# nikhilTkur/Multigrid_Nikhil_C-

Measured on AMD Instinct MI355X. Metric: fine_grid_stencil_updates_per_sec, higher is better.
Workload: dtype f64

## Files before the change

multigrid_nikhil_c-_amd/csrc/mgx.hip:

```cpp

#include "../../include/mgx.h"
#include "mgx_bottom.hpp"
#include "mgx_kernels.hpp"
#include "mgx_launch.hpp"
#include "mgx_var.hpp"
#include "mgx_galerkin.hpp"
#include "mgx_opdep.hpp"
#include "mgx_cheby.hpp"
#include "mgx_line.hpp"
#include "mgx_colour.hpp"
#include "mgx_small.hpp"
#include "mgx_krylov.hpp"
#include "mgx_refine.hpp"
#include "mgx_refine_gcr.hpp"
#include "mgx_multi.hpp"
#include "mgx_eig.hpp"
#include "mgx_eig_many.hpp"
#include "mgx_dist_plan.hpp"

#include <chrono>
#include <unistd.h>
#include <cmath>
#include <cstdio>
#include <cstdlib>
#include <cstring>
#include <string>
#include <vector>

namespace {

using namespace mgx;

thread_local std::string g_create_error;

void log_runtime_libs(const char* where)
{
    if (env_int("MGX_LOG_RUNTIME_LIBS", 0) == 0) return;
    char buf[8192];
    if (mgx_runtime_libs(buf, sizeof buf) >= 0)
        std::fprintf(stderr, "[mgx] runtime libraries mapped at %s (pid %d):\n%s", where, (int)getpid(), buf);
}

struct Level {
    int L = 0, N = 0, rows = 0;
    long pitch = 0;
    size_t bytes = 0;
    bool f64 = true;
    void *u = nullptr, *b = nullptr, *tmp = nullptr, *r = nullptr;
    void* A[9] = {};
    void* J[9] = {};
    void* wt[8] = {nullptr, nullptr, nullptr, nullptr, nullptr, nullptr, nullptr, nullptr};
    bool nine = false;
    bool stencil_set = false;
    void* cheb = nullptr;
    double lambda_g = 0.0;
    void *line_m[2] = {nullptr, nullptr}, *line_g[2] = {nullptr, nullptr}, *line_hf = nullptr, *line_hb = nullptr;
    int line_R = 0;
    size_t esize() const { return f64 ? 8 : 4; }
};

struct EventPair { hipEvent_t a, b; int cls; long long launches; long long sweeps; hipEvent_t a_use; };

}

struct mgx_solver {
    mgx_config cfg{};
    hipStream_t stream = nullptr;
    std::vector<Level> lv;
    Level fine64;
    bool mixed = false;
    bool work_f64 = true;
    BottomDST bottom;
    double* partial = nullptr;
    long partial_cap = 0;
    double* sum_dev = nullptr;
    double* sum_host = nullptr;
    std::string err;
    int rows_per_chunk = 0;
    FuseCfg fuse{10, 0, 256, 10, 10, 1024, 10, 10};
    std::vector<EventPair> ev_used, ev_free;
    double prof_ms[MGX_PROF_COUNT] = {0};
    long long prof_launches[MGX_PROF_COUNT] = {0};
    long long prof_sweeps[MGX_PROF_COUNT] = {0};
    int last_smooth_launches = 0;
    int fold = 1;
    int use_zero_in = 1;
    int norm_blocks_ready = 0;
    double fine_updates = 0.0;
    struct CycleGraph {
        std::vector<void*> before, after;
        hipGraphExec_t exec = nullptr;
        double fine_updates = 0.0;
    };
    std::vector<CycleGraph> graphs;
    int use_graph = 1;
    bool prof_mute = false;
    bool prof_chain = false;
    hipEvent_t chain_ev = nullptr;
    int mixed_fuse = 1;
    double *var_M = nullptr, *var_inv = nullptr, *var_pm = nullptr, *var_pi = nullptr;
    bool var = false;
    bool galerkin = false;
    bool gal_built = false;
    int cycle = MGX_CYCLE_V;
    int small_visit = 1;
    int small_max_n = kSmallMaxN;
    int line_dirs = 0;
    int colour = 0;
    int gs_fused = 1;
    int* line_flag = nullptr;
    int transfer = MGX_TRANSFER_BILINEAR;
    struct KrylovWs {
        void *x = nullptr, *b = nullptr;
        void *p[2] = {nullptr, nullptr}, *q = nullptr;
        void *Z[kGcrMaxRestart] = {}, *Q[kGcrMaxRestart] = {};
        double* part = nullptr;
        long part_cap = 0;
        double *sc = nullptr, *sc_host = nullptr;
        int vecs(mgx_solver* s, std::initializer_list<void**> vs, size_t bytes);
        int shared(mgx_solver* s, size_t bytes, int blocks);
        void free();
    } kry;
    struct mgx_dist* dist = nullptr;
    mgx_solver* shadow = nullptr;
    long long op_gen = 0, shadow_gen = -1;
    bool own_stream = true;
    struct MultiWs {
        struct Grids { void *u[MGX_MAX_RHS] = {}, *tmp[MGX_MAX_RHS] = {}, *b[MGX_MAX_RHS] = {}, *r[MGX_MAX_RHS] = {}; };
        std::vector<Grids> lv;
        double* part[MGX_MAX_RHS] = {};
        double *sums = nullptr, *sums_host = nullptr;
        int cols = 0;
        void* x[MGX_MAX_RHS] = {};
        void *Z[MGX_MAX_RHS][kGcrMaxRestart] = {}, *Q[MGX_MAX_RHS][kGcrMaxRestart] = {};
        double* gpart[MGX_MAX_RHS] = {};
        double *gsc = nullptr, *gsc_host = nullptr;
    } multi;
    struct EigWs {
        void *X[MGX_MAX_RHS] = {}, *AX[MGX_MAX_RHS] = {}, *AW[MGX_MAX_RHS] = {}, *P[MGX_MAX_RHS] = {}, *AP[MGX_MAX_RHS] = {};
        double *gpart = nullptr, *gsum = nullptr, *gsum_host = nullptr;
        int cols = 0;
    } eig;
    struct EigManyWs {
        void* Y[MGX_EIGS_MAX] = {};
        void** ytab = nullptr;
        double *coef = nullptr, *part = nullptr;
        int slots = 0;
    } eigm;

    int fail(int code, const std::string& m) { err = m; return code; }
};

namespace {

#define HIPCHK(h, expr)                                                                  \
    do {                                                                                 \
        hipError_t e__ = (expr);                                                         \
        if (e__ != hipSuccess)                                                           \
            return (h)->fail(MGX_ERR_HIP, std::string(#expr) + ": " + hipGetErrorString(e__)); \
    } while (0)

struct Prof {
    mgx_solver* s; int idx = -1;
    Prof(mgx_solver* s_, int cls, long long launches, bool on = true) : s(s_)
    {
        static const bool mute_all = env_int("MGX_PROF_MUTE", 0) != 0;
        if (!on || !s->cfg.profile || s->prof_mute || mute_all) return;
        EventPair p;
        if (!s->ev_free.empty()) { p = s->ev_free.back(); s->ev_free.pop_back(); }
        else {
            static const unsigned flags = env_int("MGX_PROF_EVENT_FLAGS", 1) ? hipEventDisableSystemFence : hipEventDefault;
            if (hipEventCreateWithFlags(&p.a, flags) != hipSuccess || hipEventCreateWithFlags(&p.b, flags) != hipSuccess) return;
        }
        p.cls = cls; p.launches = launches; p.sweeps = 0;
        p.a_use = p.a;
        if (s->prof_chain && s->chain_ev) p.a_use = s->chain_ev;
        else (void)hipEventRecord(p.a, s->stream);
        s->ev_used.push_back(p);
        idx = (int)s->ev_used.size() - 1;
    }
    void set(long long launches, long long sweeps)
    {
        if (idx >= 0) { s->ev_used[idx].launches = launches; s->ev_used[idx].sweeps = sweeps; }
    }
    ~Prof()
    {
        if (idx < 0) return;
        (void)hipEventRecord(s->ev_used[idx].b, s->stream);
        if (s->prof_chain) s->chain_ev = s->ev_used[idx].b;
    }
};

int prof_collect(mgx_solver* s)
{
    if (s->ev_used.empty()) return MGX_OK;
    HIPCHK(s, hipStreamSynchronize(s->stream));
    for (auto& p : s->ev_used) {
        float ms = 0.f;
        if (hipEventElapsedTime(&ms, p.a_use, p.b) == hipSuccess) {
            s->prof_ms[p.cls] += ms;
            s->prof_launches[p.cls] += p.launches;
            s->prof_sweeps[p.cls] += p.sweeps;
        }
        s->ev_free.push_back(p);
    }
    s->ev_used.clear();
    s->chain_ev = nullptr;
    return MGX_OK;
}

template <typename T>
__global__ void k_fill_rhs(T* b, int N, long pitch, int kind, double f)
{
    const int c = blockIdx.x * blockDim.x + threadIdx.x;
    const int r = blockIdx.y;
    if (c > N || r > N) return;
    const double h = 1.0 / (double)N;
    double v = 0.0;
    if (r >= 1 && r < N && c >= 1 && c < N) {
        if (kind == 0) v = f * h * h;
        else v = h * h * 8.0 * 9.869604401089358 * sinpi(2.0 * c * h) * sinpi(2.0 * r * h);
    }
    b[(long)r * pitch + c] = (T)v;
}

__device__ inline uint64_t splitmix64(uint64_t x)
{
    x += 0x9E3779B97F4A7C15ULL;
    x = (x ^ (x >> 30)) * 0xBF58476D1CE4E5B9ULL;
    x = (x ^ (x >> 27)) * 0x94D049BB133111EBULL;
    return x ^ (x >> 31);
}

template <typename T>
__global__ void k_fill_random(T* u, int N, long pitch, uint64_t seed)
{
    const int c = blockIdx.x * blockDim.x + threadIdx.x;
    const int r = blockIdx.y;
    if (c > N || r > N) return;
    double v = 0.0;
    if (r >= 1 && r < N && c >= 1 && c < N) {
        const uint64_t idx = (uint64_t)(r - 1) * (uint64_t)(N - 1) + (uint64_t)(c - 1);
        const uint64_t x = splitmix64(seed ^ splitmix64(idx));
        v = (double)(x >> 11) * (1.0 / 4503599627370496.0) - 1.0;
    }
// ... 503 lines not shown
    return fold_eligible(s, s->lv[level], s->cfg.mu1, false, 1, true);
}

bool smooth_folded(mgx_solver* s, int level, int mu, bool pre, int post, bool zero_in = false, bool coarse_zero_in = false)
{
    Level& l = s->lv[level];
    if (!fold_eligible(s, l, mu, pre, post)) return false;
    const bool fine = (level == s->cfg.finest_level);
    const bool rbgs = (s->cfg.smoother == MGX_SMOOTHER_RBGS);
    if (!l.f64 && !rbgs && mu == 10 && l.N > s->fuse.tile_max_n && post == 2 && pre &&
        cycle_k_supported(mu, false, false, 0, pre, s->fuse.arith) && !cycle_k_supported(mu, false, false, post, pre, s->fuse.arith))
        post = 0;
    {
        Prof p(s, fine ? MGX_PROF_SMOOTH_FINE : MGX_PROF_COARSE, mu);
        const Level& c = s->lv[level - 1];
        const int dt = l.f64 ? MGX_DTYPE_F64 : MGX_DTYPE_F32;
        const mgx_slab cs{level - 1, dt, c.rows, 0, s->cfg.arith};
        void* czero = (post == 1 && coarse_zero_in) ? nullptr : c.u;
        const BlockReq q = level_req(s, l, mu, pre, post, zero_in, env_int("MGX_ROWS", 0));
        int launches = 0;
        const int nb = with_kernel_set(l.f64, s->cfg.smoother, s->fuse.arith, [&](auto k) {
            using K = decltype(k);
            using T = typename K::T;
            return fold_block<T, K::SM, K::AR>(s->fuse, q, (T*)l.u, (const T*)l.b, (T*)l.tmp, l.pitch, s->cfg.omega, &cs,
                                               pre ? (const T*)c.u : nullptr, post == 1 ? (T*)c.b : nullptr, (T*)czero, 1, c.N,
                                               s->cfg.restrict_mode, s->partial, s->stream, &launches);
        });
        if (nb < 0) return false;
        if (launches & 1) std::swap(l.u, l.tmp);
        p.set(launches, mu);
        if (post == 2) s->norm_blocks_ready = nb;
    }
    if (fine) s->fine_updates += (double)mu * (double)(l.N - 1) * (double)(l.N - 1);
    return true;
}

void smooth_t(mgx_solver* s, Level& l, int mu)
{
    int launches = 0;
    with_kernel_set(l.f64, s->cfg.smoother, s->fuse.arith, [&](auto k) {
        using K = decltype(k);
        using T = typename K::T;
        (void)fold_block<T, K::SM, K::AR>(s->fuse, level_req(s, l, mu, false, 0, false, s->rows_per_chunk), (T*)l.u, (const T*)l.b,
                                          (T*)l.tmp, l.pitch, s->cfg.omega, nullptr, nullptr, nullptr, nullptr, 0, 0, 0, nullptr,
                                          s->stream, &launches);
    });
    s->last_smooth_launches = launches;
    if (launches & 1) std::swap(l.u, l.tmp);
}

void smooth(mgx_solver* s, int level, int mu, bool post = false, const MultiSet& a = kOwnSet, double* fu = nullptr)
{
    if (mu <= 0) return;
    Level& l = s->lv[level];
    const bool fine = (level == s->cfg.finest_level);
    Prof p(s, fine ? MGX_PROF_SMOOTH_FINE : MGX_PROF_COARSE, mu, own(a));
    if (s->var) smooth_var(s, level, a, mu, post);
    else smooth_t(s, l, mu);
    p.set(s->last_smooth_launches, mu);
    if (!fine) return;
    const double updates = (double)(s->line_dirs == 3 ? 2 * mu : mu) * (double)(l.N - 1) * (double)(l.N - 1);
    if (own(a)) s->fine_updates += updates;
    else if (fu) for (int j = 0; j < a.m; ++j) fu[a.act[j]] += updates;
}

void restrict_level(mgx_solver* s, int level, bool fused, bool zero_guess, const MultiSet& a = kOwnSet)
{
    Level& f = s->lv[level];
    Level& c = s->lv[level - 1];
    const bool fine = (level == s->cfg.finest_level);
    Prof p(s, fine ? MGX_PROF_RESTRICT_FINE : MGX_PROF_COARSE, 1, own(a));
    const int rpc = s->rows_per_chunk;
    const int mode = s->cfg.restrict_mode;
    with_float_type(f.f64, [&](auto tag) {
        using T = decltype(tag);
        const SetPtrs<const T> uf = set_ptrs<const T>(s, level, a, kU), bf = set_ptrs<const T>(s, level, a, kB);
        const SetPtrs<T> cb = set_ptrs<T>(s, level - 1, a, kB);
        const SetPtrs<T> cz = zero_guess ? set_ptrs<T>(s, level - 1, a, kU) : SetPtrs<T>{};
        if (opdep(s)) {
            const Launch g = make_launch(c.N, VecOf<T>::W, c.N - 1, 1);
            const T rscale = (mode == MGX_RESTRICT_FW16) ? (T)0.25 : (T)1;
            const dim3 grd(g.blocks), blk(kBlock);
            if (!fused) hipLaunchKernelGGL((k_restrict_opdep<T, 0>), grd, blk, 0, s->stream, uf.p[0], bf.p[0], op9_of<T>(f), wt8_of<T>(c), cb.p[0],
                                           cz.p[0], c.N, f.pitch, c.pitch, g.strips, rscale);
            else with_point_count(f.nine, [&](auto nq) {
                constexpr int MODE = decltype(nq)::value == 9 ? 2 : 1;
                if (a.m == 1) hipLaunchKernelGGL((k_restrict_opdep<T, MODE>), grd, blk, 0, s->stream, uf.p[0], bf.p[0], op9_of<T>(f), wt8_of<T>(c),
                                                 cb.p[0], cz.p[0], c.N, f.pitch, c.pitch, g.strips, rscale);
                else with_count<kMultiMax, 2>(a.m, [&](auto kc) {
                    constexpr int K = decltype(kc)::value;
                    hipLaunchKernelGGL((k_restrict_opdep_multi<T, MODE, K>), grd, blk, 0, s->stream, columns_in<K>(uf.p), columns_in<K>(bf.p),
                                       op9_of<T>(f), wt8_of<T>(c), columns_out<K>(cb.p), columns_out<K>(cz.p), c.N, f.pitch, c.pitch, g.strips, rscale);
                });
            });
            return;
        }
        const bool grid_residual = fused && (s->var || mode >= MGX_RESTRICT_INJECT);
        if (grid_residual) {
            if (s->var) residual_set<T, 0>(s, level, a);
            else residual_level<0>(s, f, f.u, f.b, f.r);
        }
        const SetPtrs<const T> src = grid_residual ? set_ptrs<const T>(s, level, a, kR) : bf;
        for (int j = 0; j < a.m; ++j) {
            if (mode >= MGX_RESTRICT_INJECT) {
                const double w = (mode == MGX_RESTRICT_INJECT4) ? 4.0 : 1.0;
                const dim3 blk(256), grd((c.N + 255) / 256, c.N - 1);
                hipLaunchKernelGGL((k_restrict_inject<T>), grd, blk, 0, s->stream, src.p[j], cb.p[j], cz.p[j], c.N, f.pitch, c.pitch, (T)w);
            } else {
                launch_restrict<T>(uf.p[j], src.p[j], cb.p[j], cz.p[j], f.N, f.pitch, c.pitch, 1, c.N, 0, mode, fused && !grid_residual, rpc, s->stream);
            }
        }
    });
}

void prolong_level(mgx_solver* s, int level, bool add, const MultiSet& a = kOwnSet)
{
    Level& f = s->lv[level];
    Level& c = s->lv[level - 1];
    const bool fine = (level == s->cfg.finest_level);
    Prof p(s, fine ? MGX_PROF_PROLONG_FINE : MGX_PROF_COARSE, 1, own(a));
    with_float_type(f.f64, [&](auto tag) {
        using T = decltype(tag);
        const SetPtrs<T> v = set_ptrs<T>(s, level, a, kU);
        const SetPtrs<const T> e = set_ptrs<const T>(s, level - 1, a, kU);
        if (opdep(s)) launch_prolong_opdep<T>(a.m, add, v.p, e.p, wt8_of<T>(c), c.N, f.pitch, c.pitch, s->stream);
        else for (int j = 0; j < a.m; ++j) launch_prolong<T>(v.p[j], e.p[j], f.N, f.pitch, c.pitch, 1, f.N, 0, add, s->rows_per_chunk, s->stream);
    });
}

void bottom_solve(mgx_solver* s, const MultiSet& a = kOwnSet)
{
    const int level = s->cfg.coarsest_level;
    Level& l = s->lv[level];
    Prof p(s, (l.L == s->cfg.finest_level) ? MGX_PROF_SMOOTH_FINE : MGX_PROF_COARSE, 4, own(a));
    const int n = l.N - 1;
    with_float_type(l.f64, [&](auto tag) {
        using T = decltype(tag);
        const SetPtrs<const T> b = set_ptrs<const T>(s, level, a, kB);
        const SetPtrs<T> u = set_ptrs<T>(s, level, a, kU);
        if (s->var) launch_var_dense_solve<T>(s->var_inv, a.m, b.p, u.p, n, l.pitch, s->stream);
        else s->bottom.solve<T>(b.p[0], u.p[0], l.pitch, s->stream);
    });
}

int zero_u(mgx_solver* s, int level, const MultiSet& a = kOwnSet)
{
    for (int j = 0; j < a.m; ++j) HIPCHK(s, hipMemsetAsync(slot(s, level, a.act[j], kU), 0, s->lv[level].bytes, s->stream));
    return MGX_OK;
}

bool descend(mgx_solver* s, int level, bool zero_in_here, const MultiSet& a = kOwnSet, double* fu = nullptr)
{
    const bool zin_next = own(a) && zero_in_ok(s, level - 1);
    if (!own(a) || !smooth_folded(s, level, s->cfg.mu1, false, 1, zero_in_here, zin_next)) {
        if (zero_in_here) (void)zero_u(s, level, a);
        smooth(s, level, s->cfg.mu1, false, a, fu);
        restrict_level(s, level, true, !zin_next, a);
    }
    return zin_next;
}

void ascend(mgx_solver* s, int level, int post, const MultiSet& a = kOwnSet, double* fu = nullptr)
{
    if (!own(a) || !smooth_folded(s, level, s->cfg.mu2, true, post)) {
        prolong_level(s, level, true, a);
        smooth(s, level, s->cfg.mu2, true, a, fu);
    }
}

void vcycle(mgx_solver* s, int level, bool zero_in_here = false, int post_top = 0, int kind = -1, const MultiSet& a = kOwnSet,
            double* fu = nullptr);

bool small_level(const mgx_solver* s, int level, const MultiSet& a)
{
    if (!own(a) || !s->small_visit || s->cycle == MGX_CYCLE_V || !s->galerkin || !s->gal_built) return false;
    if (s->cfg.smoother != MGX_SMOOTHER_JACOBI) return false;
    if (level <= s->cfg.coarsest_level || level >= s->cfg.finest_level) return false;
    const Level& l = s->lv[level];
    return l.nine && l.N <= s->small_max_n;
}

void small_visit(mgx_solver* s, int level, bool ascend, bool descend)
{
    Level& f = s->lv[level];
    Level& c = s->lv[level - 1];
    Prof p(s, MGX_PROF_COARSE, 1);
    with_float_type(f.f64, [&](auto tag) {
        using T = decltype(tag);
        SmallVisit<T> a;
        a.u = (T*)f.u; a.b = (const T*)f.b;
        a.a = op9_of<T>(f); a.r = jac9_of<T>(f); a.dinv = (const T*)f.J[0];
        a.cu = (T*)c.u; a.cb = (T*)c.b;
        a.w = wt8_of<T>(c);
        a.N = f.N; a.pitch = f.pitch; a.cpitch = c.pitch;
        a.ascend = ascend; a.descend = descend; a.mu1 = s->cfg.mu1; a.mu2 = s->cfg.mu2;
        a.opdep = opdep(s);
        a.omega = (T)s->cfg.omega;
        a.rc = (T)(1.0 - (double)a.omega);
        const bool fw16 = s->cfg.restrict_mode == MGX_RESTRICT_FW16;
        a.rscale = fw16 ? (T)0.25 : (T)1;
        a.wgt = fw16 ? (T)0.0625 : (T)0.25;
        launch_small_visit<T>(a, s->stream);
    });
    p.set(1, (ascend ? s->cfg.mu2 : 0) + (descend ? s->cfg.mu1 : 0));
}

void coarse_visits(mgx_solver* s, int level, bool zero_in_here, int kind, const MultiSet& a = kOwnSet, double* fu = nullptr)
{
    const bool twice = kind != MGX_CYCLE_V && level > s->cfg.coarsest_level;
    const int second = kind == MGX_CYCLE_F ? MGX_CYCLE_V : kind;
    if (twice && small_level(s, level, a)) {
        small_visit(s, level, false, true);
        coarse_visits(s, level - 1, false, kind);
        small_visit(s, level, true, true);
        coarse_visits(s, level - 1, false, second);
        small_visit(s, level, true, false);
        return;
    }
    vcycle(s, level, zero_in_here, 0, kind, a, fu);
    if (twice) vcycle(s, level, false, 0, second, a, fu);
}

void vcycle(mgx_solver* s, int level, bool zero_in_here, int post_top, int kind, const MultiSet& a, double* fu)
{
    if (kind < 0) kind = s->cycle;
    if (level == s->cfg.coarsest_level) {
        if (s->cfg.bottom == MGX_BOTTOM_EXACT) {
            bottom_solve(s, a);
        } else {
            smooth(s, level, s->cfg.mu1, false, a, fu);
            smooth(s, level, s->cfg.mu2, true, a, fu);
        }
        return;
    }
    if (small_level(s, level, a)) {
        small_visit(s, level, false, true);
        coarse_visits(s, level - 1, false, kind);
        small_visit(s, level, true, false);
        return;
    }
    const bool zin_next = descend(s, level, zero_in_here, a, fu);
    coarse_visits(s, level - 1, zin_next, kind, a, fu);
    ascend(s, level, post_top, a, fu);
}

int fmg(mgx_solver* s)
{
    const int lo = s->cfg.coarsest_level, hi = s->cfg.finest_level;
    for (int l = hi; l > lo; --l) restrict_level(s, l, false, false);
    if (s->cfg.bottom == MGX_BOTTOM_EXACT) {
        bottom_solve(s);
    } else {
        int rc = zero_u(s, lo);
        if (rc) return rc;
        for (int i = 0; i <= s->cfg.mu0; ++i) vcycle(s, lo);
    }
    for (int l = lo + 1; l <= hi; ++l) {
        prolong_level(s, l, false);
        for (int i = 0; i <= s->cfg.mu0; ++i) vcycle(s, l);
    }
    return MGX_OK;
}

int enqueue_norm(mgx_solver* s, const Level& l, const void* u, const void* b, int cls)
{
    if (s->norm_blocks_ready > 0 && u == s->lv[s->cfg.finest_level].u && !s->mixed) {
        Prof p(s, cls, 1);
        hipLaunchKernelGGL(k_reduce_partials, dim3(1), dim3(kReduceThreads), 0, s->stream, s->partial, s->norm_blocks_ready,
                           s->sum_dev);
    } else {
        Prof p(s, cls, 2);
        residual_level<1>(s, l, u, b, nullptr);
    }
    s->norm_blocks_ready = 0;
    HIPCHK(s, hipMemcpyAsync(s->sum_host, s->sum_dev, sizeof(double), hipMemcpyDeviceToHost, s->stream));
    return MGX_OK;
}

int residual_norm_grid(mgx_solver* s, const Level& l, const void* u, const void* b, double* out, int cls)
{
    int rc = enqueue_norm(s, l, u, b, cls);
    if (rc) return rc;
    HIPCHK(s, hipStreamSynchronize(s->stream));
    *out = std::sqrt(*s->sum_host);
    return MGX_OK;
}

constexpr size_t kMaxGraphs = 8;

std::vector<void*> buffer_state(const mgx_solver* s)
{
    std::vector<void*> v;
    for (int l = s->cfg.coarsest_level; l <= s->cfg.finest_level; ++l) { v.push_back(s->lv[l].u); v.push_back(s->lv[l].tmp); }
    return v;
}

void set_buffer_state(mgx_solver* s, const std::vector<void*>& v)
{
    size_t i = 0;
    for (int l = s->cfg.coarsest_level; l <= s->cfg.finest_level; ++l) { s->lv[l].u = v[i++]; s->lv[l].tmp = v[i++]; }
}

template <typename Body>
hipGraphExec_t cached_graph(mgx_solver* s, unsigned tag, Body&& enqueue)
{
    std::vector<void*> key = buffer_state(s);
    key.push_back(reinterpret_cast<void*>((uintptr_t)tag));
    for (auto& c : s->graphs)
        if (c.before == key) {
            set_buffer_state(s, c.after);
            s->fine_updates += c.fine_updates;
            return c.exec;
        }
    if (s->graphs.size() >= kMaxGraphs) return nullptr;
    const double fu0 = s->fine_updates;
    hipGraph_t graph = nullptr;
    hipGraphExec_t exec = nullptr;
    hipError_t e = hipStreamBeginCapture(s->stream, hipStreamCaptureModeThreadLocal);
    if (e == hipSuccess) {
        s->prof_mute = true;
        const int rc = enqueue();
        s->prof_mute = false;
        e = hipStreamEndCapture(s->stream, &graph);
        if (e == hipSuccess && rc != MGX_OK) e = hipErrorUnknown;
        if (e == hipSuccess) e = hipGraphInstantiate(&exec, graph, nullptr, nullptr, 0);
        if (graph) (void)hipGraphDestroy(graph);
    }
    if (e != hipSuccess) {
        (void)hipGetLastError();
        set_buffer_state(s, key);
        s->fine_updates = fu0;
        s->use_graph = 0;
        return nullptr;
    }
    s->graphs.push_back({key, buffer_state(s), exec, s->fine_updates - fu0});
    return exec;
}

int coarse_part_graph(mgx_solver* s, int level, bool zero_in_here)
{
    auto body = [&] { coarse_visits(s, level, zero_in_here, s->cycle); return MGX_OK; };
    const hipGraphExec_t exec = cached_graph(s, 4u | (zero_in_here ? 8u : 0u), body);
    if (!exec) return body();
    Prof p(s, MGX_PROF_COARSE, 1);
    HIPCHK(s, hipGraphLaunch(exec, s->stream));
    return MGX_OK;
}

int zero_start_u(mgx_solver* s, bool* implicit)
{
    const int L = s->cfg.finest_level;
    const bool one_level = L == s->cfg.coarsest_level;
    *implicit = zero_in_ok(s, L);
    if (*implicit) return MGX_OK;
    if (one_level && !s->mixed) return MGX_OK;
    return zero_u(s, L);
}

int enqueue_cycle(mgx_solver* s, bool want_norm, bool zero_start, bool split)
{
    struct Chain {
        mgx_solver* s;
        Chain(mgx_solver* s_, bool on) : s(s_) { s->prof_chain = on && env_int("MGX_PROF_CHAIN", 1) != 0; s->chain_ev = nullptr; }
        ~Chain() { s->prof_chain = false; s->chain_ev = nullptr; }
    } chain(s, split);
    const int L = s->cfg.finest_level;
    const int post = want_norm ? 2 : 0;
    s->norm_blocks_ready = 0;
    bool zin = false;
    if (zero_start)
        if (int rc = zero_start_u(s, &zin)) return rc;
    if (split) {
        const bool zin_next = descend(s, L, zin);
        if (int rc = coarse_part_graph(s, L - 1, zin_next)) return rc;
        ascend(s, L, post);
    } else {
        vcycle(s, L, zin, post);
    }
    return want_norm ? enqueue_norm(s, s->lv[L], s->lv[L].u, s->lv[L].b, MGX_PROF_NORM_FINE) : MGX_OK;
}

int cycle_body(mgx_solver* s, bool want_norm, bool zero_start, double* r)
{
    const bool split = s->cfg.profile == 2 && s->use_graph && !s->mixed && s->cfg.finest_level > s->cfg.coarsest_level;
    const bool whole = s->use_graph && !s->cfg.profile && !s->mixed;
    auto body = [&] { return enqueue_cycle(s, want_norm, zero_start, split); };
    const hipGraphExec_t exec = whole ? cached_graph(s, (want_norm ? 1u : 0u) | (zero_start ? 2u : 0u), body) : nullptr;
    if (exec) {
        s->norm_blocks_ready = 0;
        HIPCHK(s, hipGraphLaunch(exec, s->stream));
    } else if (int rc = body()) {
        return rc;
    }
    if (!want_norm) return MGX_OK;
    HIPCHK(s, hipStreamSynchronize(s->stream));
    *r = std::sqrt(*s->sum_host);
    return MGX_OK;
}

void finish_solve(mgx_stats* stats, double* history, int history_cap, const std::vector<double>& hist, int cycles, bool converged,
                  std::chrono::steady_clock::time_point t0, double fine_updates)
{
    if (stats) {
        stats->cycles = cycles;
        stats->initial_residual = hist.front();
        stats->final_residual = hist.back();
        stats->converged = converged ? 1 : 0;
        stats->seconds = std::chrono::duration<double>(std::chrono::steady_clock::now() - t0).count();
        stats->fine_updates = fine_updates;
        stats->history_len = (int)hist.size();
    }
    if (history)
        for (int i = 0; i < (int)hist.size() && i < history_cap; ++i) history[i] = hist[i];
}

double pow2_floor(double x)
{
    int e;
    (void)std::frexp(x, &e);
    return std::ldexp(1.0, e - 1);
}

Level* pick(mgx_solver* s, int level, int which, void** grid)
{
    Level* l = &s->lv[level];
    if (s->mixed && level == s->cfg.finest_level) l = &s->fine64;
    switch (which) {
        case MGX_VEC_U: *grid = l->u; break;
        case MGX_VEC_B: *grid = l->b; break;
        case MGX_VEC_R: *grid = l->r; break;
        default: *grid = nullptr;
    }
    return l;
}

template <typename T>
void fold_ring(std::vector<T>& b, const T* ring, size_t n)
{
    const size_t N = n + 1;
    const T* top = ring;
    const T* bot = ring + (N + 1);
    const T* lef = ring + 2 * (N + 1);
    const T* rig = lef + (N - 1);
    for (size_t j = 0; j < n; ++j) {
        b[j] += top[j + 1];
        b[(n - 1) * n + j] += bot[j + 1];
    }
    for (size_t i = 0; i < n; ++i) {
        b[i * n] += lef[i];
        b[i * n + (n - 1)] += rig[i];
    }
}

template <typename Enqueue>
int time_on_stream(mgx_solver* s, double* ms, Enqueue enqueue)
{
    hipEvent_t a = nullptr, b = nullptr;
    auto timed = [&]() -> int {
        HIPCHK(s, hipEventCreate(&a));
        HIPCHK(s, hipEventCreate(&b));
        HIPCHK(s, hipEventRecord(a, s->stream));
        enqueue();
        HIPCHK(s, hipEventRecord(b, s->stream));
        HIPCHK(s, hipEventSynchronize(b));
        HIPCHK(s, hipGetLastError());
        float f = 0.f;
        HIPCHK(s, hipEventElapsedTime(&f, a, b));
        *ms = f;
        return MGX_OK;
    };
    const int rc = timed();
    if (a) (void)hipEventDestroy(a);
    if (b) (void)hipEventDestroy(b);
    return rc;
}

}

#include "mgx_dist.hpp"

#define NO_DIST(s)                                                                        \
    if ((s)->dist) return (s)->fail(MGX_ERR_STATE, "not available on a multi-GPU handle (see mgx.h, Multi-GPU)");

#include "mgx_krylov_host.hpp"
#include "mgx_multi_host.hpp"

static int create_solver(const mgx_config* cfg, const mgx_solver* like, mgx_handle* out);

#include "mgx_refine_host.hpp"
#include "mgx_multi_refine_host.hpp"
#include "mgx_eig_host.hpp"
#include "mgx_eig_many_host.hpp"

extern "C" {

int mgx_config_default(mgx_config* c)
{
    if (!c) return MGX_ERR_INVALID;
    c->finest_level = 10;
    c->coarsest_level = 7;
    c->mu0 = 30;
    c->mu1 = 10;
    c->mu2 = 10;
    c->omega = 2.0 / 3.0;
    c->smoother = MGX_SMOOTHER_JACOBI;
    c->dtype = MGX_DTYPE_F64;
    c->schedule = MGX_SCHEDULE_FMG;
    c->restrict_mode = MGX_RESTRICT_CONSISTENT;
    c->bottom = MGX_BOTTOM_EXACT;
    c->device = 0;
    c->profile = 0;
    c->n_gpus = 0;
    c->cut_level = 0;
    for (int i = 0; i < MGX_MAX_GPUS; ++i) c->devices[i] = -1;
    c->arith = MGX_ARITH_SEPARATE;
    c->op = MGX_OPERATOR_POISSON;
    return MGX_OK;
}

const char* mgx_status_string(int st)
{
    switch (st) {
        case MGX_OK: return "ok";
        case MGX_ERR_INVALID: return "invalid argument";
        case MGX_ERR_NO_DEVICE: return "no usable HIP device";
        case MGX_ERR_HIP: return "HIP runtime error";
        case MGX_ERR_ALLOC: return "device allocation failed";
        case MGX_ERR_STATE: return "invalid state";
        default: return "unknown status";
    }
}

const char* mgx_last_error(mgx_handle h) { return h ? h->err.c_str() : g_create_error.c_str(); }

int mgx_level_n(int level) { return (level >= 1 && level < 31) ? (1 << level) - 1 : -1; }

long mgx_level_pitch(int level, int dtype)
{
    if (level < 1 || level > 20 || (dtype != MGX_DTYPE_F32 && dtype != MGX_DTYPE_F64)) return -1;
    return level_pitch(level, dtype);
}

static int create_solver(const mgx_config* cfg, const mgx_solver* like, mgx_handle* out)
{
    if (!cfg || !out) { g_create_error = "null argument"; return MGX_ERR_INVALID; }
    *out = nullptr;
    if (cfg->coarsest_level < 2 || cfg->finest_level < cfg->coarsest_level || cfg->finest_level > 15 ||
        cfg->mu0 < 0 || cfg->mu1 < 0 || cfg->mu2 < 0 || !(cfg->omega > 0.0 && cfg->omega < 2.0) ||
        cfg->smoother < 0 || cfg->smoother > MGX_SMOOTHER_COLOR_SGS || cfg->smoother == 3 || cfg->smoother == 7 || cfg->dtype < 0 || cfg->dtype > 2 ||
        cfg->schedule < 0 || cfg->schedule > 1 || cfg->restrict_mode < 0 || cfg->restrict_mode > MGX_RESTRICT_INJECT4 ||
        cfg->bottom < 0 || cfg->bottom > 1 || cfg->arith < 0 || cfg->arith > 1 || (cfg->op != MGX_OPERATOR_POISSON && cfg->op != MGX_OPERATOR_STENCIL5 && cfg->op != MGX_OPERATOR_GALERKIN)) {
        g_create_error = "invalid configuration";
        return MGX_ERR_INVALID;
    }
    const bool galerkin = (cfg->op == MGX_OPERATOR_GALERKIN);
    const bool var = (cfg->op == MGX_OPERATOR_STENCIL5) || galerkin;
    if (cfg->bottom == MGX_BOTTOM_EXACT && cfg->coarsest_level > (var ? 5 : 8)) {
        g_create_error = var ? "exact bottom solve of a general operator (dense inverse) supports coarsest_level <= 5"
                             : "exact bottom solve supports coarsest_level <= 8";
        return MGX_ERR_INVALID;
    }
    const bool cheby = (cfg->smoother == MGX_SMOOTHER_CHEBYSHEV);
    if (cheby && !var) {
        g_create_error = "MGX_SMOOTHER_CHEBYSHEV: op = MGX_OPERATOR_STENCIL5 or MGX_OPERATOR_GALERKIN only (the constant stencil has its fused and folded passes)";
        return MGX_ERR_INVALID;
    }
    const bool line = (cfg->smoother >= MGX_SMOOTHER_LINE_X && cfg->smoother <= MGX_SMOOTHER_LINE_ALT);
    const bool colour = (cfg->smoother == MGX_SMOOTHER_COLOR_GS || cfg->smoother == MGX_SMOOTHER_COLOR_SGS);
    if (colour && (!var || cfg->dtype == MGX_DTYPE_MIXED || cfg->arith != MGX_ARITH_SEPARATE || cfg->n_gpus > 1)) {
        g_create_error = "MGX_SMOOTHER_COLOR_GS / COLOR_SGS: op = MGX_OPERATOR_STENCIL5 or MGX_OPERATOR_GALERKIN, dtype F64 or F32, arith SEPARATE, one GPU";
        return MGX_ERR_INVALID;
    }
    if (line && (!var || cfg->dtype == MGX_DTYPE_MIXED || cfg->arith != MGX_ARITH_SEPARATE || cfg->n_gpus > 1)) {
        g_create_error = "MGX_SMOOTHER_LINE_X / LINE_Y / LINE_ALT: op = MGX_OPERATOR_STENCIL5 or MGX_OPERATOR_GALERKIN, dtype F64 or F32, arith SEPARATE, one GPU";
        return MGX_ERR_INVALID;
    }
    if (var && (cfg->dtype == MGX_DTYPE_MIXED || cfg->smoother == MGX_SMOOTHER_RBGS || cfg->arith != MGX_ARITH_SEPARATE || cfg->n_gpus > 1)) {
// ... 369 lines not shown

int mgx_set_coefficient(mgx_handle s, const double* a_nodes, size_t count)
{
    if (!s || !a_nodes) return MGX_ERR_INVALID;
    NO_DIST(s)
    if (!s->var) return s->fail(MGX_ERR_STATE, "handle was created with op = MGX_OPERATOR_POISSON");
    const int Lf = s->cfg.finest_level, Nf = 1 << Lf;
    if (count != (size_t)(Nf + 1) * (size_t)(Nf + 1)) return s->fail(MGX_ERR_INVALID, "coefficient must hold (N + 1)^2 nodal values, N = 2^finest_level");
    double* dev = nullptr;
    if (hipMalloc(&dev, count * sizeof(double)) != hipSuccess) return s->fail(MGX_ERR_ALLOC, "hipMalloc failed for the nodal coefficient");
    int rc = MGX_OK;
    if (hipMemcpyAsync(dev, a_nodes, count * sizeof(double), hipMemcpyHostToDevice, s->stream) != hipSuccess) rc = s->fail(MGX_ERR_HIP, "copy of the nodal coefficient failed");
    for (int lv = s->galerkin ? Lf : s->cfg.coarsest_level; lv <= Lf && rc == MGX_OK; ++lv) {
        Level& l = s->lv[lv];
        const dim3 blk(256), grd((l.N + 1 + 255) / 256, l.N + 1);
        const int q = 1 << (Lf - lv);
        with_float_type(l.f64, [&](auto tag) {
            using T = decltype(tag);
            hipLaunchKernelGGL((k_var_from_nodes<T>), grd, blk, 0, s->stream, dev, Nf, q, out9(op9_of<T>(l)), l.N, l.pitch);
        });
        if (!s->galerkin) rc = var_build(s, l);
    }
    if (hipStreamSynchronize(s->stream) != hipSuccess && rc == MGX_OK) rc = s->fail(MGX_ERR_HIP, "sampling the nodal coefficient failed");
    (void)hipFree(dev);
    if (s->galerkin && rc == MGX_OK) { s->lv[Lf].nine = false; galerkin_invalidate(s); }
    return rc;
}

int mgx_get_stencil(mgx_handle s, int level, int which, void* dst, size_t count)
{
    if (!s || !dst) return MGX_ERR_INVALID;
    NO_DIST(s)
    if (!s->var) return s->fail(MGX_ERR_STATE, "handle was created with op = MGX_OPERATOR_POISSON");
    if (!level_ok(s, level) || which < 0 || which > 9) return s->fail(MGX_ERR_INVALID, "level or array selector out of range");
    Level& l = s->lv[level];
    if (l.nine) return s->fail(MGX_ERR_STATE, "nine-point operator (a coarse level, or a nine-point finest level, of a GALERKIN handle): use mgx_get_stencil9");
    if (!l.stencil_set) return s->fail(MGX_ERR_STATE, "operator of this level not set");
    if (s->galerkin && which >= 5 && !s->gal_built) return s->fail(MGX_ERR_STATE, "Galerkin hierarchy not built (mgx_build_galerkin)");
    return copy_out(s, l, which < 5 ? l.A[which] : l.J[which - 5], dst, count);
}

int mgx_build_galerkin(mgx_handle s)
{
    if (!s) return MGX_ERR_INVALID;
    NO_DIST(s)
    if (!s->galerkin) return s->fail(MGX_ERR_STATE, "handle was not created with op = MGX_OPERATOR_GALERKIN");
    if (!s->lv[s->cfg.finest_level].stencil_set)
        return s->fail(MGX_ERR_STATE, "finest operator not set (mgx_set_stencil / mgx_set_coefficient / mgx_set_stencil9 / mgx_set_tensor)");
    return s->work_f64 ? galerkin_build_t<double>(s, MGX_TRANSFER_BILINEAR) : galerkin_build_t<float>(s, MGX_TRANSFER_BILINEAR);
}

int mgx_build_galerkin_transfer(mgx_handle s, int transfer)
{
    if (!s) return MGX_ERR_INVALID;
    NO_DIST(s)
    if (!s->galerkin) return s->fail(MGX_ERR_STATE, "handle was not created with op = MGX_OPERATOR_GALERKIN");
    if (transfer != MGX_TRANSFER_BILINEAR && transfer != MGX_TRANSFER_OPERATOR)
        return s->fail(MGX_ERR_INVALID, "transfer must be MGX_TRANSFER_BILINEAR or MGX_TRANSFER_OPERATOR");
    if (!s->lv[s->cfg.finest_level].stencil_set)
        return s->fail(MGX_ERR_STATE, "finest operator not set (mgx_set_stencil / mgx_set_coefficient / mgx_set_stencil9 / mgx_set_tensor)");
    return s->work_f64 ? galerkin_build_t<double>(s, transfer) : galerkin_build_t<float>(s, transfer);
}

int mgx_get_transfer(mgx_handle s, int* transfer)
{
    if (!s || !transfer) return MGX_ERR_INVALID;
    NO_DIST(s)
    if (!s->galerkin) return s->fail(MGX_ERR_STATE, "handle was not created with op = MGX_OPERATOR_GALERKIN");
    if (!s->gal_built) return s->fail(MGX_ERR_STATE, "Galerkin hierarchy not built (mgx_build_galerkin)");
    *transfer = s->transfer;
    return MGX_OK;
}

int mgx_get_lambda_max(mgx_handle s, int level, double* out)
{
    if (!s || !out) return MGX_ERR_INVALID;
    NO_DIST(s)
    if (!s->var) return s->fail(MGX_ERR_STATE, "handle was created with op = MGX_OPERATOR_POISSON (g = 2 for the constant stencil)");
    if (!level_ok(s, level)) return s->fail(MGX_ERR_INVALID, "level out of range");
    if (s->galerkin && !s->gal_built) return s->fail(MGX_ERR_STATE, "Galerkin hierarchy not built (mgx_build_galerkin)");
    if (!s->lv[level].stencil_set) return s->fail(MGX_ERR_STATE, "operator of this level not set");
    *out = s->lv[level].lambda_g;
    return MGX_OK;
}

int mgx_get_line_factor(mgx_handle s, int level, int dir, int which, void* dst, size_t count)
{
    if (!s || !dst) return MGX_ERR_INVALID;
    NO_DIST(s)
    if (!s->line_dirs) return s->fail(MGX_ERR_STATE, "handle was not created with a line smoother (MGX_SMOOTHER_LINE_X / LINE_Y / LINE_ALT)");
    if (!level_ok(s, level) || dir < 0 || dir > 1 || which < 0 || which > 1) return s->fail(MGX_ERR_INVALID, "level, direction or array selector out of range");
    if (!(s->line_dirs & (1 << dir))) return s->fail(MGX_ERR_STATE, dir == 0 ? "the handle's smoother has no x-lines (MGX_SMOOTHER_LINE_Y)" : "the handle's smoother has no y-lines (MGX_SMOOTHER_LINE_X)");
    if (s->galerkin && !s->gal_built) return s->fail(MGX_ERR_STATE, "Galerkin hierarchy not built (mgx_build_galerkin)");
    if (!s->lv[level].stencil_set) return s->fail(MGX_ERR_STATE, "operator of this level not set");
    Level& l = s->lv[level];
    return copy_out(s, l, which == 0 ? l.line_m[dir] : l.line_g[dir], dst, count);
}

int mgx_get_line_chunks(mgx_handle s, int level, int* rows, int* chunks)
{
    if (!s || !rows || !chunks) return MGX_ERR_INVALID;
    NO_DIST(s)
    if (!(s->line_dirs & 2)) return s->fail(MGX_ERR_STATE, "the handle's smoother has no y-lines (MGX_SMOOTHER_LINE_Y / LINE_ALT)");
    if (!level_ok(s, level)) return s->fail(MGX_ERR_INVALID, "level out of range");
    *rows = s->lv[level].line_R;
    *chunks = line_chunks(s->lv[level].N, s->lv[level].line_R);
    return MGX_OK;
}

int mgx_get_prolongation(mgx_handle s, int level, int which, void* dst, size_t count)
{
    if (!s || !dst) return MGX_ERR_INVALID;
    NO_DIST(s)
    if (!s->galerkin) return s->fail(MGX_ERR_STATE, "handle was not created with op = MGX_OPERATOR_GALERKIN");
    if (level <= s->cfg.coarsest_level || level > s->cfg.finest_level || which < 0 || which > 7)
        return s->fail(MGX_ERR_INVALID, "level or array selector out of range");
    if (!s->gal_built) return s->fail(MGX_ERR_STATE, "Galerkin hierarchy not built (mgx_build_galerkin)");
    if (s->transfer != MGX_TRANSFER_OPERATOR)
        return s->fail(MGX_ERR_STATE, "the hierarchy was built with MGX_TRANSFER_BILINEAR: its weights are 1/2 and 1/4 and are not stored");
    Level& c = s->lv[level - 1];
    return copy_out(s, c, c.wt[which], dst, count);
}

int mgx_get_stencil9(mgx_handle s, int level, int which, void* dst, size_t count)
{
    if (!s || !dst) return MGX_ERR_INVALID;
    NO_DIST(s)
    if (!s->galerkin) return s->fail(MGX_ERR_STATE, "handle was not created with op = MGX_OPERATOR_GALERKIN");
    if (!level_ok(s, level) || which < 0 || which > 17) return s->fail(MGX_ERR_INVALID, "level or array selector out of range");
    if (!s->gal_built) return s->fail(MGX_ERR_STATE, "Galerkin hierarchy not built (mgx_build_galerkin)");
    Level& l = s->lv[level];
    const void* src = which < 9 ? l.A[which] : l.J[which - 9];
    const int slot = which < 9 ? which : which - 9;
    if (!src || (!l.nine && slot >= 5)) {
        const size_t n = (size_t)l.N - 1;
        if (count != n * n) return s->fail(MGX_ERR_INVALID, "vector length must be n*n with n = 2^level - 1");
        std::memset(dst, 0, count * l.esize());
        return MGX_OK;
    }
    return copy_out(s, l, src, dst, count);
}

#define MIXED_GUARD(lvl)                                                                  \
    if (s->mixed && (lvl) == s->cfg.finest_level)                                         \
        return s->fail(MGX_ERR_STATE, "dtype MIXED: operators and schedules are not defined on the finest level " \
                                      "(double data, float inner cycle); use mgx_solve, or a F64 / F32 handle");

#define OP_PROLOGUE(lvl_min)                                                              \
    if (!s) return MGX_ERR_INVALID;                                                       \
    NO_DIST(s)                                                                            \
    if (level < (lvl_min) || level > s->cfg.finest_level)                                 \
        return s->fail(MGX_ERR_INVALID, "level out of range for this operator");          \
    MIXED_GUARD(level)                                                                    \
    if (int vr__ = var_ready(s, s->cfg.coarsest_level, level)) return vr__;

#define OP_EPILOGUE                                                                       \
    HIPCHK(s, hipGetLastError());                                                         \
    HIPCHK(s, hipStreamSynchronize(s->stream));                                           \
    return MGX_OK;

int mgx_smooth(mgx_handle s, int level, int mu)
{
    OP_PROLOGUE(s->cfg.coarsest_level)
    if (mu < 0) return s->fail(MGX_ERR_INVALID, "mu must be >= 0");
    smooth(s, level, mu);
    OP_EPILOGUE
}

int mgx_residual(mgx_handle s, int level)
{
    OP_PROLOGUE(s->cfg.coarsest_level)
    Level& l = s->lv[level];
    int rc = ensure_r(s, l);
    if (rc) return rc;
    residual_level<0>(s, l, l.u, l.b, l.r);
    OP_EPILOGUE
}

int mgx_restrict(mgx_handle s, int level)
{
    OP_PROLOGUE(s->cfg.coarsest_level + 1)
    restrict_level(s, level, true, true);
    OP_EPILOGUE
}

int mgx_restrict_rhs(mgx_handle s, int level)
{
    OP_PROLOGUE(s->cfg.coarsest_level + 1)
    restrict_level(s, level, false, false);
    OP_EPILOGUE
}

int mgx_prolong_add(mgx_handle s, int level)
{
    OP_PROLOGUE(s->cfg.coarsest_level + 1)
    prolong_level(s, level, true);
    OP_EPILOGUE
}

int mgx_prolong(mgx_handle s, int level)
{
    OP_PROLOGUE(s->cfg.coarsest_level + 1)
    prolong_level(s, level, false);
    OP_EPILOGUE
}

int mgx_bottom_solve(mgx_handle s)
{
    if (!s) return MGX_ERR_INVALID;
    NO_DIST(s)
    if (s->cfg.bottom != MGX_BOTTOM_EXACT) return s->fail(MGX_ERR_STATE, "handle was created with bottom = SMOOTH");
    MIXED_GUARD(s->cfg.coarsest_level)
    if (int vr = var_ready(s, s->cfg.coarsest_level, s->cfg.coarsest_level)) return vr;
    bottom_solve(s);
    OP_EPILOGUE
}

int mgx_residual_norm(mgx_handle s, int level, double* out)
{
    if (!s || !out) return MGX_ERR_INVALID;
    if (!level_ok(s, level)) return s->fail(MGX_ERR_INVALID, "level out of range");
    if (s->dist) {
        if (level != s->cfg.finest_level) return s->fail(MGX_ERR_STATE, "multi-GPU handles: residual norm of the finest level only");
        return dist_norm(s, s->dist, out);
    }
    if (int vr = var_ready(s, level, level)) return vr;
    void* gu = nullptr; void* gb = nullptr;
    Level* l = pick(s, level, MGX_VEC_U, &gu);
    (void)pick(s, level, MGX_VEC_B, &gb);
    return residual_norm_grid(s, *l, gu, gb, out, level == s->cfg.finest_level ? MGX_PROF_NORM_FINE : MGX_PROF_COARSE);
}

int mgx_vcycle(mgx_handle s, int level)
{
    if (s && s->dist) {
        if (level != s->cfg.finest_level) return s->fail(MGX_ERR_STATE, "multi-GPU handles: V-cycles from the finest level only");
        int rc = dist_vcycle(s, s->dist);
        return rc ? rc : dist_sync(s, s->dist);
    }
    OP_PROLOGUE(s->cfg.coarsest_level)
    vcycle(s, level);
    OP_EPILOGUE
}

int mgx_set_cycle(mgx_handle s, int cycle)
{
    if (!s) return MGX_ERR_INVALID;
    if (cycle != MGX_CYCLE_V && cycle != MGX_CYCLE_W && cycle != MGX_CYCLE_F)
        return s->fail(MGX_ERR_INVALID, "cycle must be MGX_CYCLE_V, MGX_CYCLE_W or MGX_CYCLE_F");
    if (s->dist) return s->fail(MGX_ERR_STATE, "mgx_set_cycle: multi-GPU handles run V-cycles only (the slab plan has no second coarse visit)");
    if (s->mixed) return s->fail(MGX_ERR_STATE, "mgx_set_cycle: dtype MIXED handles run V-cycles only; use a F64 or F32 handle");
    if (!s->var)
        return s->fail(MGX_ERR_STATE, "mgx_set_cycle: op = MGX_OPERATOR_POISSON handles run V-cycles only; W- and F-cycles are for "
                                      "MGX_OPERATOR_STENCIL5 and MGX_OPERATOR_GALERKIN");
    drop_graphs(s);
    s->cycle = cycle;
    if (s->shadow) { drop_graphs(s->shadow); s->shadow->cycle = cycle; }
    return MGX_OK;
}

int mgx_get_cycle(mgx_handle s, int* cycle)
{
    if (!s) return MGX_ERR_INVALID;
    if (!cycle) return s->fail(MGX_ERR_INVALID, "null argument");
    *cycle = s->cycle;
    return MGX_OK;
}

int mgx_vcycle_zero(mgx_handle s)
{
    if (!s) return MGX_ERR_INVALID;
    NO_DIST(s)
    MIXED_GUARD(s->cfg.finest_level)
    if (int vr = var_ready(s, s->cfg.coarsest_level, s->cfg.finest_level)) return vr;
    double unused = 0.0;
    int rc = cycle_body(s, false, true, &unused);
    if (rc) return rc;
    OP_EPILOGUE
}

int mgx_fmg(mgx_handle s)
{
    if (!s) return MGX_ERR_INVALID;
    if (s->dist) {
        int rc = dist_fmg(s, s->dist);
        return rc ? rc : dist_sync(s, s->dist);
    }
    MIXED_GUARD(s->cfg.finest_level)
    if (int vr = var_ready(s, s->cfg.coarsest_level, s->cfg.finest_level)) return vr;
    int rc = fmg(s);
    if (rc) return rc;
    OP_EPILOGUE
}

int mgx_solve(mgx_handle s, double tol, int max_cycles, mgx_stats* stats, double* history, int history_cap)
{
    if (!s || max_cycles < 0 || !(tol >= 0.0)) return MGX_ERR_INVALID;
    if (s->dist) return dist_solve(s, s->dist, tol, max_cycles, stats, history, history_cap);
    if (int vr = var_ready(s, s->cfg.coarsest_level, s->cfg.finest_level)) return vr;
    const int L = s->cfg.finest_level;
    const bool do_fmg = (s->cfg.schedule == MGX_SCHEDULE_FMG);
    std::vector<double> hist;
    hist.reserve(max_cycles + 1);
    s->fine_updates = 0.0;
    HIPCHK(s, hipStreamSynchronize(s->stream));
    const auto t0 = std::chrono::steady_clock::now();
    int rc = MGX_OK;
    double r = 0.0;
    int k = 0;

    if (!s->mixed) {
        Level& l = s->lv[L];
        if ((rc = residual_norm_grid(s, l, l.u, l.b, &r, MGX_PROF_NORM_FINE))) return rc;
        hist.push_back(r);
        for (k = 0; k < max_cycles; ++k) {
            if (hist[k] <= tol * hist[0]) break;
            s->norm_blocks_ready = 0;
            if (k == 0 && do_fmg) {
                if ((rc = fmg(s))) return rc;
                if ((rc = residual_norm_grid(s, l, l.u, l.b, &r, MGX_PROF_NORM_FINE))) return rc;
            } else if ((rc = cycle_body(s, true, false, &r))) {
                return rc;
            }
            hist.push_back(r);
        }
    } else {
        Level& w = s->lv[L];
        Level& d = s->fine64;
        const double n = (double)(w.N - 1);
        const int rpc = s->rows_per_chunk;
        if ((rc = residual_norm_grid(s, d, d.u, d.b, &r, MGX_PROF_NORM_FINE))) return rc;
        hist.push_back(r);
        for (k = 0; k < max_cycles; ++k) {
            if (hist[k] <= tol * hist[0]) break;
            const Launch g = make_launch(d.N, 2, d.N - 1, rpc);
            double pending_scale = 0.0;
            if (k == 0 && do_fmg) {
                HIPCHK(s, hipMemsetAsync(d.u, 0, d.bytes, s->stream));
                double bn = 0.0;
                if ((rc = residual_norm_grid(s, d, d.u, d.b, &bn, MGX_PROF_NORM_FINE))) return rc;
                const double scale = pow2_floor(bn / n);
                hipLaunchKernelGGL(k_scale_f64_to_f32, dim3(g.blocks), dim3(kBlock), 0, s->stream, (float*)w.b,
                                   (const double*)d.b, 1.0 / scale, d.N, d.pitch, w.pitch, 1, d.N, g.R, g.strips, g.chunks);
                if ((rc = fmg(s))) return rc;
                hipLaunchKernelGGL(k_axpy_f32_to_f64, dim3(g.blocks), dim3(kBlock), 0, s->stream, (double*)d.u,
                                   (const float*)w.u, scale, d.N, d.pitch, w.pitch, 1, d.N, g.R, g.strips, g.chunks, 1);
            } else {
                const double scale = pow2_floor(hist[k > 0 ? k - 1 : 0] / n);
                if (k == 0) {
                    Prof p(s, MGX_PROF_NORM_FINE, 2);
                    launch_residual<double, 2>((const double*)d.u, (const double*)d.b, w.b, w.pitch, s->partial,
                                               s->sum_dev, 1.0 / scale, d.N, d.pitch, 1, d.N, rpc, s->stream, s->partial_cap, d.rows);
                }
                double unused = 0.0;
                if ((rc = cycle_body(s, false, true, &unused))) return rc;
                pending_scale = scale;
                if (!(s->mixed_fuse && d.tmp)) {
                    hipLaunchKernelGGL(k_axpy_f32_to_f64, dim3(g.blocks), dim3(kBlock), 0, s->stream, (double*)d.u,
                                       (const float*)w.u, scale, d.N, d.pitch, w.pitch, 1, d.N, g.R, g.strips, g.chunks, 0);
                    pending_scale = 0.0;
                }
            }
            {
                const double next_scale = pow2_floor(hist[k] / n);
                Prof p(s, MGX_PROF_NORM_FINE, 2);
                if (pending_scale != 0.0) {
// ... 678 lines not shown
```

multigrid_nikhil_c-_amd/csrc/mgx_geom.hpp:

```cpp
#pragma once

#if defined(__HIPCC__)
#define MGX_GEOM_HD __host__ __device__ __forceinline__
#else
#define MGX_GEOM_HD inline
#endif

namespace mgx {

constexpr int kGeomWavesPerBlock = 4;
constexpr int kGeomCusPerXcd = 32;
constexpr int kGeomResidentBlocks = 512;

struct CycleGeom {
    int R, Re, Rl;
    int Rf;
    int chunks, chunks_e;
    int row_last0;
    int RB, n_tall, n_short;
    long waves;
    int blocks;
};

struct CTile { int strip, r0, r1; bool active; };

MGX_GEOM_HD int geom_min(int a, int b) { return a < b ? a : b; }

MGX_GEOM_HD CTile cycle_tile_at(int block, int wave, int grid, int strips, int chunks, int chunks_e, int R, int Re, int row_lo,
                                int row_hi, int row_last0, int Rl, int RB, int n_tall, int n_short, int Rf)
{
    const int per_xcd = grid >> 3;
    const int xcd = block & 7;
    const int nth = block >> 3;
    const int si = strips - 2;
    CTile t;
    t.strip = 0; t.r0 = 0; t.r1 = 0; t.active = false;
    if (row_last0 != 0) {
        const int n_edge = 3 * si + 2 * chunks_e;
        int e = -1, m = -1, s = -1;
        if (n_tall > 0) {
            const int n_f = n_edge + n_tall * si, n_s = n_short * si;
            const int pf = (n_f + 7) >> 3, ps = (n_s + 7) >> 3;
            if (nth < kGeomCusPerXcd) {
                const int lw = nth * kGeomWavesPerBlock + wave;
                const int f = xcd * pf + lw;
                if (lw < pf && f < n_f) { if (f < n_edge) e = f; else m = f - n_edge; }
            } else {
                const int lw = (nth - kGeomCusPerXcd) * kGeomWavesPerBlock + wave;
                if (lw < ps && xcd * ps + lw < n_s) s = xcd * ps + lw;
            }
        } else {
            const int n_mid = (chunks - 3) * si;
            const int pe = (n_edge + 7) >> 3, pm = (n_mid + 7) >> 3;
            const int lw = nth * kGeomWavesPerBlock + wave;
            if (lw < pe) { if (xcd * pe + lw < n_edge) e = xcd * pe + lw; }
            else if (lw - pe < pm && xcd * pm + (lw - pe) < n_mid) m = xcd * pm + (lw - pe);
        }
        if (e >= 0) {
            t.active = true;
            if (e < 3 * si) {
                const int which = e / si;
                t.strip = 1 + (e - which * si);
                t.r0 = which == 0 ? row_lo : (which == 1 ? row_last0 : row_last0 + Rl);
                t.r1 = which == 0 ? row_lo + Rf : (which == 1 ? row_last0 + Rl : row_hi);
            } else {
                const int k = e - 3 * si;
                const int chunk = k >> 1;
                t.strip = (k & 1) ? strips - 1 : 0;
                t.r0 = row_lo + chunk * Re;
                t.r1 = geom_min(t.r0 + Re, row_hi);
            }
        } else if (m >= 0) {
            const int chunk = m / si;
            t.active = true;
            t.strip = 1 + (m - chunk * si);
            t.r0 = row_lo + Rf + chunk * R;
            t.r1 = geom_min(t.r0 + R, row_last0);
        } else if (s >= 0) {
            const int chunk = s / si;
            t.active = true;
            t.strip = 1 + (s - chunk * si);
            t.r0 = row_lo + Rf + n_tall * R + chunk * RB;
            t.r1 = geom_min(t.r0 + RB, row_last0);
        }
        t.active = t.active && t.r0 < t.r1;
        return t;
    }
    const int b = xcd * per_xcd + (xcd >= 4 ? per_xcd - 1 - nth : nth);
    const long g = (long)b * kGeomWavesPerBlock + wave;
    const long n_int = si > 0 ? (long)chunks * si : 0;
    if (g < n_int) {
        const int chunk = (int)(g / si);
        t.strip = 1 + (int)(g - (long)chunk * si);
        t.r0 = row_lo + chunk * R;
        t.r1 = geom_min(t.r0 + R, row_hi);
        t.active = t.r0 < t.r1;
    } else {
        const long e = g - n_int;
        int chunk;
        if (si > 0) { chunk = (int)(e >> 1); t.strip = (e & 1) ? strips - 1 : 0; }
        else { chunk = (int)(e / strips); t.strip = (int)(e - (long)chunk * strips); }
        t.r0 = row_lo + chunk * Re;
        t.r1 = geom_min(t.r0 + Re, row_hi);
        t.active = chunk < chunks_e && t.r0 < row_hi;
    }
    return t;
}


inline int trip_rows(int R, int extra, int trip, int step)
{
    int best = -1;
    for (int r = R; r < R + 2 * trip; r += step) {
        const int m = (r + extra) % trip;
        if (m == 0) return r;
        if (m == trip - 1 && best < 0) best = r;
    }
    return best < 0 ? R : best;
}

inline int edge_rows_pct(int R, int extra, int trip, int pct)
{
    const double frac = 0.01 * (double)pct;
    const int k = (int)(frac * (double)(R + extra) / (double)trip + 0.5);
    const int Re = R - k * trip;
    return Re >= trip ? Re : (R >= 2 * trip ? trip : R);
}

struct GeomKnobs {
    int edge_short = 1;
    int edge_pct = 23;
    int last_pct = 38;
    int min_chunk = 16;
    int min_rounds = 1;
    int min_rounds_rows = 1024;
    int pair = 1;
    int pair_ratio = 130;
    int pair_max_rows = 640;
    int pair_min_rows = 150;
};

inline int geom_blocks(const CycleGeom& g, int strips)
{
    int blocks = (int)(((g.waves + kGeomWavesPerBlock - 1) / kGeomWavesPerBlock + 7) / 8 * 8);
    if (g.row_last0 != 0) {
        const int si = strips - 2;
        const int n_edge = 3 * si + 2 * g.chunks_e;
        if (g.n_tall > 0) {
            const int ps = (g.n_short * si + 7) / 8;
            blocks = 8 * (kGeomCusPerXcd + (ps + kGeomWavesPerBlock - 1) / kGeomWavesPerBlock);
        } else {
            const int pe = (n_edge + 7) / 8, pm = ((g.chunks - 3) * si + 7) / 8;
            blocks = 8 * ((pe + pm + kGeomWavesPerBlock - 1) / kGeomWavesPerBlock);
        }
    }
    return blocks;
}

inline CycleGeom cycle_geom(int row_lo, int row_hi, int strips, int R, int Re, int Rl, int Rf = -1)
{
    const int rows = row_hi - row_lo;
    if (Rf < 0) Rf = Re;
    CycleGeom g;
    g.R = R; g.Re = Re; g.Rl = Rl; g.Rf = Rf; g.RB = 0; g.n_tall = 0; g.n_short = 0;
    g.chunks_e = (rows + Re - 1) / Re;
    if ((Re >= R && Rf >= R && Rl >= R) || rows <= Rf + 2 * Rl + 2 || strips < 3) {
        g.R = (Re >= R) ? R : Re; g.Re = g.R; g.Rl = g.R; g.Rf = g.R;
        g.row_last0 = 0;
        g.chunks = g.chunks_e = (rows + g.R - 1) / g.R;
    } else {
        const int last = row_hi - Rl + ((row_hi - Rl - row_lo) & 1);
        g.row_last0 = last - Rl;
        g.chunks = 3 + (g.row_last0 - (row_lo + Rf) + R - 1) / R;
    }
    g.waves = strips > 2 ? (long)g.chunks * (strips - 2) + 2L * g.chunks_e : (long)g.chunks_e * strips;
    g.blocks = geom_blocks(g, strips);
    return g;
}

inline bool cycle_geom_paired(int row_lo, int row_hi, int strips, int extra, int trip, const GeomKnobs& kn, bool top_edge, bool bot_edge,
                              CycleGeom* out)
{
    const int rows = row_hi - row_lo;
    const int si = strips - 2;
    if (si < 1) return false;
    const int slots = kGeomCusPerXcd * kGeomWavesPerBlock;
    for (int rb = trip_rows(kn.min_chunk, extra, trip, 2); rb <= kn.pair_max_rows; rb += trip) {
        const int steps_b = (rb + extra + trip - 1) / trip * trip;
        const int steps_a = (int)(((long)steps_b * kn.pair_ratio / 100 + trip - 1) / trip) * trip;
        const int ra = (steps_a - extra) & ~1;
        if (ra > kn.pair_max_rows) break;
        if (ra <= rb) continue;
        const int re = edge_rows_pct(ra, extra, trip, kn.edge_pct), rl = bot_edge ? edge_rows_pct(ra, extra, trip, kn.last_pct) : ra;
        const int rf = top_edge ? re : ra;
        if (rows <= rf + 2 * rl + 2 + rb) continue;
        const int chunks_e = (rows + re - 1) / re;
        const int n_edge = 3 * si + 2 * chunks_e;
        const int last = row_hi - rl + ((row_hi - rl - row_lo) & 1);
        const int row_last0 = last - rl;
        const int mid = row_last0 - (row_lo + rf);
        if (mid < rb) continue;
        const int nt_max = (8 * slots - 7 - n_edge) / si, ns_max = (8 * slots - 7) / si;
        if (nt_max < 1 || ns_max < 1) continue;
        if ((long)nt_max * ra + (long)ns_max * rb < mid) continue;
        if (rb < kn.pair_min_rows) return false;
        int nt = (int)((double)mid * ((double)nt_max * ra / ((double)nt_max * ra + (double)ns_max * rb)) / ra + 0.5);
        if (nt > nt_max) nt = nt_max;
        while (nt > 0 && (long)nt * ra > mid - rb) --nt;
        int ns = nt > 0 ? (mid - nt * ra + rb - 1) / rb : ns_max + 1;
        while (ns > ns_max && nt < nt_max && (long)(nt + 1) * ra <= mid - rb) { ++nt; ns = (mid - nt * ra + rb - 1) / rb; }
        if (nt < 1 || ns > ns_max) continue;
        const int pf = (n_edge + nt * si + 7) / 8, ps = (ns * si + 7) / 8;
        if (pf > slots || ps > slots) continue;
        CycleGeom g;
        g.R = ra; g.Re = re; g.Rl = rl; g.Rf = rf; g.RB = rb; g.n_tall = nt; g.n_short = ns;
        g.chunks_e = chunks_e; g.row_last0 = row_last0; g.chunks = 3 + nt + ns;
        g.waves = (long)g.chunks * si + 2L * chunks_e;
        g.blocks = geom_blocks(g, strips);
        if (g.blocks > kGeomResidentBlocks) continue;
        *out = g;
        return true;
    }
    return false;
}

inline CycleGeom cycle_geom_pick(int row_lo, int row_hi, int strips, int extra, int trip, int R, bool auto_rows, bool deep,
                                 const GeomKnobs& kn, bool top_edge = true, bool bot_edge = true)
{
    if (R & 1) ++R;
    R = trip_rows(R, extra, trip, 2);
    CycleGeom g = cycle_geom(row_lo, row_hi, strips, R, R, R);
    if (!deep) return g;
    auto shaped = [&](int r) {
        return cycle_geom(row_lo, row_hi, strips, r, kn.edge_short ? edge_rows_pct(r, extra, trip, kn.edge_pct) : r,
                          (kn.edge_short && bot_edge) ? edge_rows_pct(r, extra, trip, kn.last_pct) : r,
                          (kn.edge_short && top_edge) ? edge_rows_pct(r, extra, trip, kn.edge_pct) : r);
    };
    if (!auto_rows) return kn.edge_short ? shaped(R) : g;
    if (kn.pair && kn.edge_short && strips >= 3) {
        CycleGeom p;
        if (cycle_geom_paired(row_lo, row_hi, strips, extra, trip, kn, top_edge, bot_edge, &p)) return p;
    }
    bool found = false;
    for (int m = (row_hi - row_lo >= kn.min_rounds_rows ? kn.min_rounds : 1); m <= 64 && !found; ++m) {
        for (int r = trip_rows(kn.min_chunk, extra, trip, 2); r <= 204; r += trip) {
            const CycleGeom c = shaped(r);
            if (c.waves <= 2048L * m && c.blocks <= kGeomResidentBlocks * m) { g = c; found = true; break; }
        }
    }
    return g;
}

constexpr int kTileWideWaves = 8;

struct TileWideGeom {
    int He, Hx;
    int TH, TW;
    int tiles_y, tiles_x;
};

MGX_GEOM_HD TileWideGeom tile_wide_geom(int N, int row_lo, int row_hi, int He, int W, int RW)
{
    TileWideGeom g;
    g.He = He;
    g.Hx = (He + W - 1) / W * W;
    g.TH = kTileWideWaves * RW - 2 * He;
    g.TW = 64 * W - 2 * g.Hx;
    g.tiles_y = (g.TH > 0 && row_hi > row_lo) ? (row_hi - row_lo + g.TH - 1) / g.TH : 0;
    g.tiles_x = g.TW > 0 ? (N + g.TW - 1) / g.TW : 0;
    return g;
}

MGX_GEOM_HD int tile_wide_rw(int N, int short_max_n) { return N <= short_max_n ? 8 : 10; }

}
```

multigrid_nikhil_c-_amd/csrc/mgx_inst.hip:

```cpp
#include "mgx_launch.hpp"
#if MGX_INST_KIND == 4
#include "mgx_cheby.hpp"
#elif MGX_INST_KIND == 5
#include "mgx_small.hpp"
#elif MGX_INST_KIND == 6
#include "mgx_line.hpp"
#elif MGX_INST_KIND == 7
#include "mgx_krylov.hpp"
#elif MGX_INST_KIND == 8
#include "mgx_colour.hpp"
#elif MGX_INST_KIND == 9
#include "mgx_multi.hpp"
#elif MGX_INST_KIND == 10
#include "mgx_refine_gcr.hpp"
#elif MGX_INST_KIND == 11
#include "mgx_eig.hpp"
#elif MGX_INST_KIND == 12
#include "mgx_eig_many.hpp"
#endif

namespace mgx {
using T_ = MGX_INST_T;
#if MGX_INST_KIND == 1
#if MGX_INST_PP == 0
#define PP_ 1, 2
#elif MGX_INST_PP == 1
#define PP_ 1, 0
#elif MGX_INST_PP == 2
#define PP_ 0, 1
#elif MGX_INST_PP == 3
#define PP_ 0, 2
#else
#define PP_ 1, 1
#endif
template int launch_cycle<T_, PP_, MGX_INST_SM, MGX_INST_AR>(int, const T_*, const T_*, T_*, const FoldArgs&, int, long, T_, T_, int, hipStream_t);
#elif MGX_INST_KIND == 2
template bool launch_fused<T_, MGX_INST_SM, MGX_INST_AR>(int, const T_*, const T_*, T_*, int, long, int, int, T_, T_, int, int, int, int, hipStream_t, int, int);
#elif MGX_INST_KIND == 3
template int launch_tile_pass<T_, MGX_INST_SM, MGX_INST_AR>(const T_*, const T_*, T_*, const FoldArgs&, int, long, T_, T_, int, int, bool, int, hipStream_t);
#elif MGX_INST_KIND == 4
template void launch_cheby<T_>(const VarLevel<T_>&, const T_*, const T_*, T_*, T_*, bool, T_, T_, T_, T_, hipStream_t);
template void launch_lambda_max<T_>(const VarLevel<T_>&, double*, long, double*, hipStream_t);
#elif MGX_INST_KIND == 5
template hipError_t small_visit_prepare<T_>();
template void launch_small_visit<T_>(const SmallVisit<T_>&, hipStream_t);
#elif MGX_INST_KIND == 6
template void launch_line_factor<T_>(const LineLevel<T_>&, int, int*, hipStream_t);
template int launch_line_sweep<T_>(const LineLevel<T_>&, T_*, const T_*, int, hipStream_t);
#elif MGX_INST_KIND == 7
template void launch_gcr_orth<T_>(int, T_*, T_*, const T_*, const GcrBasis<T_>&, double*, double*, int, long, const Launch&, int, hipStream_t);
#elif MGX_INST_KIND == 8
template int launch_gs_colours<T_>(const ColourLevel<T_>&, T_*, const T_*, bool, hipStream_t);
template void launch_gs_rb<T_>(const ColourLevel<T_>&, const T_*, const T_*, T_*, bool, hipStream_t);
#elif MGX_INST_KIND == 9
template void launch_gcr_direction_multi<T_>(int, bool, const T_* const*, T_* const*, T_* const*, const Op9<T_>&, int, long, const Launch&, hipStream_t);
#elif MGX_INST_KIND == 10
#elif MGX_INST_KIND == 11
template void launch_eig_gram<T_>(int, int, bool, const T_* const*, const T_* const*, double*, double*, const EigGeom&, hipStream_t);
template void launch_eig_combine<T_>(int, int, const T_* const*, T_* const*, const double*, const EigGeom&, hipStream_t);
template void launch_eig_residual<T_>(int, const T_* const*, const T_* const*, T_* const*, double* const*, double* const*, const double*, const EigGeom&,
                                      hipStream_t);
template void launch_eig_apply<T_>(int, bool, const T_* const*, T_* const*, const Op9<T_>&, const EigGeom&, hipStream_t);
#elif MGX_INST_KIND == 12
template void launch_eig_project_dots<T_>(int, int, const T_* const*, const T_* const*, double*, double*, const EigGeom&, hipStream_t);
template void launch_eig_project_sub<T_>(int, int, const T_* const*, T_* const*, const double*, const EigGeom&, hipStream_t);
#else
#error "MGX_INST_KIND must be 1 .. 12"
#endif
}
```

multigrid_nikhil_c-_amd/csrc/mgx_kernels.hpp:

```cpp
#pragma once

#include <hip/hip_runtime.h>
#include "mgx_geom.hpp"
#include "mgx_phase_trace.hpp"
#include <stdint.h>
#include <type_traits>

namespace mgx {

template <int B, int E, typename F> __device__ __forceinline__ void static_for(F&& f)
{
    if constexpr (B < E) {
        f(std::integral_constant<int, B>{});
        static_for<B + 1, E>(f);
    }
}

constexpr int kWave = 64;
constexpr int kBlock = 256;
constexpr int kWavesPerBlock = kBlock / kWave;
constexpr int kOutLanes = kWave - 2;

template <typename T> struct VecOf;
template <> struct VecOf<double> { using type = double2; static constexpr int W = 2; };
// ... 1417 lines not shown
__global__ void __launch_bounds__(kBlock)
k_tile_smooth(const T* __restrict__ vin, const T* __restrict__ rhs, T* __restrict__ vout,
              const T* __restrict__ coarse_e, T* __restrict__ coarse_b, T* __restrict__ coarse_zero, T wgt,
              double* __restrict__ partial, int N, long pitch, long cpitch, int levels, T c0, T c1,
              int tiles_x, int zero_in, int row_lo, int row_hi, CycleWin win)
{
    constexpr int RW = kTileBand;
    __shared__ T edge[2][kWavesPerBlock][2][kWave];
    __shared__ double wsum[kWavesPerBlock];
    const int He = levels + tile_extra<POST>();
    const int TH = kTileSY - 2 * He, TW = kTileSX - 2 * He;
    const int lane = threadIdx.x & 63;
    const int wv = __builtin_amdgcn_readfirstlane(threadIdx.x >> 6);
    const int ty = blockIdx.x / tiles_x, tx = blockIdx.x - ty * tiles_x;
    const int y0 = wv * RW;
    const int gy0 = row_lo + ty * TH - He + y0;
    const int gx = 1 + tx * TW - He + lane;
    const bool colunk = gx > 0 && gx < N;
    const int NC = N / 2;

    T u[RW], b[RW];
    unsigned rowmask = 0;
#pragma unroll
    for (int i = 0; i < RW; ++i) {
        const int gy = gy0 + i;
        const bool rowok = gy > 0 && gy < N && gy >= win.row_first && gy <= win.row_last;
        if (rowok) rowmask |= 1u << i;
        const bool unk = colunk && rowok;
        const long at = (long)gy * pitch + gx;
        u[i] = (unk && !zero_in) ? vin[at] : (T)0;
        b[i] = unk ? rhs[at] : (T)0;
    }
    if (PRE) {
        const bool codd = (gx & 1) != 0;
#pragma unroll
        for (int i = 0; i < RW; ++i) {
            const int gy = gy0 + i;
            const bool rodd = (gy & 1) != 0;
            const bool unk = colunk && ((rowmask >> i) & 1u) && (gy >> 1) >= win.crow_first && (gy >> 1) + (rodd ? 1 : 0) <= win.crow_last;
            const T* e = coarse_e + (long)(gy >> 1) * cpitch + (gx >> 1);
            const T a00 = unk ? e[0] : (T)0;
            const T a01 = (unk && codd) ? e[1] : (T)0;
            const T a10 = (unk && rodd) ? e[cpitch] : (T)0;
            const T a11 = (unk && rodd && codd) ? e[cpitch + 1] : (T)0;
            const T ev = codd ? (T)0.5 * (a00 + a01) : a00;
            const T od = codd ? (T)0.25 * (((a00 + a10) + a01) + a11) : (T)0.5 * (a00 + a10);
            const T add = rodd ? od : ev;
            u[i] = unk ? u[i] + add : u[i];
        }
    }

    int buf = 0;
    auto halo_rows = [&](const T (&a)[RW], T& up, T& dn) {
        edge[buf][wv][0][lane] = a[0];
        edge[buf][wv][1][lane] = a[RW - 1];
        __syncthreads();
        up = wv > 0 ? edge[buf][wv - 1][1][lane] : (T)0;
        dn = wv < kWavesPerBlock - 1 ? edge[buf][wv + 1][0][lane] : (T)0;
        buf ^= 1;
    };
    for (int j = 1; j <= levels; ++j) {
        T up, dn;
        halo_rows(u, up, dn);
        const bool colact = colunk && lane >= j && lane < kTileSX - j;
        const int ilo = max(j - y0, 0), ihi = min(kTileSY - j - y0, RW);
        const unsigned act = ihi > ilo ? (rowmask & (((1u << (ihi - ilo)) - 1u) << ilo)) : 0u;
        T prev = up;
#pragma unroll
        for (int i = 0; i < RW; ++i) {
            const T cur = u[i];
            const T below = (i == RW - 1) ? dn : u[i + 1];
            const T l = from_left(cur), r = from_right(cur);
            const bool rowact = (act >> i) & 1u;
            if (SM == 0) {
                const T o = jac_pt<AR>(c0, cur, c1 * b[i], c1, nbr(prev, l, r, below));
                u[i] = (colact && rowact) ? o : cur;
            } else {
                const T o = (T)0.25 * (b[i] + nbr(prev, l, r, below));
                u[i] = (colact && rowact && ((gy0 + i + gx) & 1) == ((j - 1) & 1)) ? o : cur;
            }
            prev = cur;
        }
    }

    const bool colout = lane >= He && lane < He + TW && gx < N;
#pragma unroll
    for (int i = 0; i < RW; ++i) {
        const int y = y0 + i, gy = gy0 + i;
        if (y >= He && y < He + TH && gy < N && gy >= row_lo && gy < row_hi && colout) vout[(long)gy * pitch + gx] = u[i];
    }

    if (POST != 0) {
        T up, dn;
        halo_rows(u, up, dn);
        T res[RW];
        double acc = 0.0;
        T prev = up;
#pragma unroll
        for (int i = 0; i < RW; ++i) {
            const T cur = u[i];
            const T below = (i == RW - 1) ? dn : u[i + 1];
            const int y = y0 + i, gy = gy0 + i;
            const T l = from_left(cur), r = from_right(cur);
            T rr = (T)0;
            if (colunk && gy > 0 && gy < N) rr = b[i] - (-nbr(prev, l, r, below) + (T)4 * cur);
            res[i] = rr;
            if (POST == 2 && y >= He && y < He + TH && gy >= row_lo && gy < row_hi && colout) acc += (double)rr * (double)rr;
            prev = cur;
        }
        if (POST == 2) {
            for (int off = 32; off > 0; off >>= 1) acc += __shfl_down(acc, off, kWave);
            if (lane == 0) wsum[wv] = acc;
            __syncthreads();
            if (threadIdx.x == 0) {
                double sum = 0.0;
                for (int w2 = 0; w2 < kWavesPerBlock; ++w2) sum += wsum[w2];
                partial[blockIdx.x] = sum;
            }
        }
        if (POST == 1) {
            T rup, rdn;
            halo_rows(res, rup, rdn);
            const int J = gx >> 1;
            const bool cst = colout && (gx & 1) == 0 && J >= 1 && J < NC;
#pragma unroll
            for (int i = 0; i < RW; ++i) {
                const T c = res[i];
                const T n = (i == 0) ? rup : res[i - 1];
                const T s2 = (i == RW - 1) ? rdn : res[i + 1];
                const int y = y0 + i, gy = gy0 + i;
                T corners = from_left(n) + from_right(n);
                corners = corners + from_left(s2);
                corners = corners + from_right(s2);
                T edges = from_left(c) + from_right(c);
                edges = edges + n;
                edges = edges + s2;
                const T o = wgt * ((corners + (T)2 * edges) + (T)4 * c);
                if (cst && y >= He && y < He + TH && (gy & 1) == 0 && gy < N && gy >= row_lo && gy < row_hi &&
                    (gy >> 1) >= win.emit_lo && (gy >> 1) < win.emit_hi) {
                    const long at = (long)(gy >> 1) * cpitch + J;
                    coarse_b[at] = o;
                    if (coarse_zero) coarse_zero[at] = (T)0;
                }
            }
        }
    }
}

__device__ __forceinline__ double vget(const double2& v, int e) { return e == 0 ? v.x : v.y; }
__device__ __forceinline__ float vget(const float4& v, int e) { return e == 0 ? v.x : (e == 1 ? v.y : (e == 2 ? v.z : v.w)); }
__device__ __forceinline__ double2 vmake(const double (&a)[2]) { return make_double2(a[0], a[1]); }
__device__ __forceinline__ float4 vmake(const float (&a)[4]) { return make_float4(a[0], a[1], a[2], a[3]); }

template <typename T, int SM, int PRE, int POST, int AR, int RW>
__global__ void __launch_bounds__(kTileWideWaves * kWave)
k_tile_wide(const T* __restrict__ vin, const T* __restrict__ rhs, T* __restrict__ vout,
            const T* __restrict__ coarse_e, T* __restrict__ coarse_b, T* __restrict__ coarse_zero, T wgt,
            double* __restrict__ partial, int N, long pitch, long cpitch, int levels, T c0, T c1,
            int tiles_x, int zero_in, int row_lo, int row_hi, CycleWin win)
{
    using V = typename VecOf<T>::type;
    constexpr int W = VecOf<T>::W;
    constexpr int NW = kTileWideWaves;
    __shared__ V edge[2][NW][2][kWave];
    __shared__ double wsum[NW];
    MGX_PHASE_BEGIN();
    const TileWideGeom g = tile_wide_geom(N, row_lo, row_hi, levels + tile_extra<POST>(), W, RW);
    const int He = g.He, TH = g.TH, TW = g.TW;
    const int lane = threadIdx.x & 63;
    const int wv = __builtin_amdgcn_readfirstlane(threadIdx.x >> 6);
    const int ty = blockIdx.x / tiles_x, tx = blockIdx.x - ty * tiles_x;
    const int y0 = wv * RW;
    const int gy0 = row_lo + ty * TH - He + y0;
    const int cx0 = tx * TW;
    const int gx0 = cx0 - g.Hx + W * lane;
    const bool vld = gx0 >= 0 && gx0 < N;
    const bool cu0 = vld && gx0 > 0;
    bool cu[W];
#pragma unroll
    for (int e = 0; e < W; ++e) cu[e] = e == 0 ? cu0 : vld;
    const int NC = N / 2;
    MGX_PHASE_AFTER(gx0 + gy0);

    T u[RW][W], b[RW][W];
    unsigned rowmask = 0;
#pragma unroll
    for (int i = 0; i < RW; ++i) {
        const int gy = gy0 + i;
        const bool rowok = gy > 0 && gy < N && gy >= win.row_first && gy <= win.row_last;
        if (rowok) rowmask |= 1u << i;
        const long at = (long)gy * pitch + gx0;
        V uv = vzero((V*)nullptr), bv = vzero((V*)nullptr);
        if (vld && rowok) {
            bv = *reinterpret_cast<const V*>(rhs + at);
            if (!zero_in) uv = *reinterpret_cast<const V*>(vin + at);
        }
#pragma unroll
        for (int e = 0; e < W; ++e) {
            u[i][e] = cu[e] ? vget(uv, e) : (T)0;
            b[i][e] = cu[e] ? vget(bv, e) : (T)0;
        }
    }
    if (PRE) {
        constexpr int NCR = RW / 2 + 1, NCC = W / 2 + 1;
        const int kc0 = gy0 >> 1, J = gx0 >> 1;
        T cr[NCR][NCC];
#pragma unroll
        for (int k = 0; k < NCR; ++k) {
            const int cy = kc0 + k;
            const bool ok = vld && cy >= 0 && cy <= NC && cy >= win.crow_first && cy <= win.crow_last;
            const T* ep = coarse_e + (long)cy * cpitch + J;
#pragma unroll
            for (int m = 0; m < NCC; ++m) cr[k][m] = ok ? ep[m] : (T)0;
        }
        auto correct = [&](auto parity) {
            constexpr int par = decltype(parity)::value;
#pragma unroll
            for (int i = 0; i < RW; ++i) {
                const int gy = gy0 + i;
                const bool rodd = ((par + i) & 1) != 0;
                const int kr = (par + i) >> 1;
                const bool rin = ((rowmask >> i) & 1u) && (gy >> 1) >= win.crow_first && (gy >> 1) + (rodd ? 1 : 0) <= win.crow_last;
#pragma unroll
                for (int e = 0; e < W; ++e) {
                    const bool codd = (e & 1) != 0;
                    const bool unk = cu[e] && rin;
                    const T a00 = unk ? cr[kr][e >> 1] : (T)0;
                    const T a01 = (unk && codd) ? cr[kr][(e >> 1) + 1] : (T)0;
                    const T a10 = (unk && rodd) ? cr[kr + (rodd ? 1 : 0)][e >> 1] : (T)0;
                    const T a11 = (unk && rodd && codd) ? cr[kr + (rodd ? 1 : 0)][(e >> 1) + 1] : (T)0;
                    const T ev = codd ? (T)0.5 * (a00 + a01) : a00;
                    const T od = codd ? (T)0.25 * (((a00 + a10) + a01) + a11) : (T)0.5 * (a00 + a10);
                    const T add = rodd ? od : ev;
                    u[i][e] = unk ? u[i][e] + add : u[i][e];
                }
            }
        };
        if (gy0 & 1) correct(std::integral_constant<int, 1>{});
        else correct(std::integral_constant<int, 0>{});
    }

    MGX_PHASE_AFTER(b[RW - 1][W - 1]);
    MGX_PHASE_AFTER(u[RW - 1][W - 1]);

    int buf = 0;
    auto halo_rows = [&](const T (&a)[RW][W], T (&up)[W], T (&dn)[W]) {
        edge[buf][wv][0][lane] = vmake(a[0]);
        edge[buf][wv][1][lane] = vmake(a[RW - 1]);
        __syncthreads();
        const V uv = wv > 0 ? edge[buf][wv - 1][1][lane] : vzero((V*)nullptr);
        const V dv = wv < NW - 1 ? edge[buf][wv + 1][0][lane] : vzero((V*)nullptr);
#pragma unroll
        for (int e = 0; e < W; ++e) { up[e] = vget(uv, e); dn[e] = vget(dv, e); }
        buf ^= 1;
    };
    for (int j = 1; j <= levels; ++j) {
        T up[W], dn[W];
        halo_rows(u, up, dn);
        const int colour = (j - 1) & 1;
        T prev[W];
#pragma unroll
        for (int e = 0; e < W; ++e) prev[e] = up[e];
#pragma unroll
        for (int i = 0; i < RW; ++i) {
            T cur[W];
#pragma unroll
            for (int e = 0; e < W; ++e) cur[e] = u[i][e];
            const T l = from_left(cur[W - 1]), r = from_right(cur[0]);
            const bool rowact = (rowmask >> i) & 1u;
#pragma unroll
            for (int e = 0; e < W; ++e) {
                const T below = (i == RW - 1) ? dn[e] : u[i + 1][e];
                const T we = e == 0 ? l : cur[e - 1], ea = e == W - 1 ? r : cur[e + 1];
                if (SM == 0) {
                    const T o = jac_pt<AR>(c0, cur[e], c1 * b[i][e], c1, nbr(prev[e], we, ea, below));
                    u[i][e] = (cu[e] && rowact) ? o : cur[e];
                } else {
                    const T o = (T)0.25 * (b[i][e] + nbr(prev[e], we, ea, below));
                    u[i][e] = (cu[e] && rowact && ((gy0 + i + e) & 1) == colour) ? o : cur[e];
                }
            }
#pragma unroll
            for (int e = 0; e < W; ++e) prev[e] = cur[e];
        }
        MGX_PHASE_AFTER(u[RW - 1][W - 1]);
    }

    const bool colout = gx0 >= cx0 && gx0 < cx0 + TW && gx0 < N;
#pragma unroll
    for (int i = 0; i < RW; ++i) {
        const int y = y0 + i, gy = gy0 + i;
        if (y >= He && y < He + TH && gy < N && gy >= row_lo && gy < row_hi && colout)
            *reinterpret_cast<V*>(vout + (long)gy * pitch + gx0) = vmake(u[i]);
    }
    MGX_PHASE();

    if (POST != 0) {
        T up[W], dn[W];
        halo_rows(u, up, dn);
        T res[RW][W];
        double acc = 0.0;
        T prev[W];
#pragma unroll
        for (int e = 0; e < W; ++e) prev[e] = up[e];
#pragma unroll
        for (int i = 0; i < RW; ++i) {
            const int y = y0 + i, gy = gy0 + i;
            const T l = from_left(u[i][W - 1]), r = from_right(u[i][0]);
            const bool rowunk = gy > 0 && gy < N;
            const bool rowout = POST == 2 && y >= He && y < He + TH && gy >= row_lo && gy < row_hi && colout;
#pragma unroll
            for (int e = 0; e < W; ++e) {
                const T cur = u[i][e];
                const T below = (i == RW - 1) ? dn[e] : u[i + 1][e];
                const T we = e == 0 ? l : u[i][e - 1], ea = e == W - 1 ? r : u[i][e + 1];
                T rr = (T)0;
                if (cu[e] && rowunk) rr = b[i][e] - (-nbr(prev[e], we, ea, below) + (T)4 * cur);
                res[i][e] = rr;
                if (rowout) acc += (double)rr * (double)rr;
            }
#pragma unroll
            for (int e = 0; e < W; ++e) prev[e] = u[i][e];
        }
        MGX_PHASE_AFTER(res[RW - 1][W - 1]);
        if (POST == 2) {
            for (int off = 32; off > 0; off >>= 1) acc += __shfl_down(acc, off, kWave);
            if (lane == 0) wsum[wv] = acc;
            __syncthreads();
            if (threadIdx.x == 0) {
                double sum = 0.0;
                for (int w2 = 0; w2 < NW; ++w2) sum += wsum[w2];
                partial[blockIdx.x] = sum;
            }
        }
        if (POST == 1) {
            T rup[W], rdn[W];
            halo_rows(res, rup, rdn);
#pragma unroll
            for (int i = 0; i < RW; ++i) {
                const int y = y0 + i, gy = gy0 + i;
                const bool rowst = y >= He && y < He + TH && (gy & 1) == 0 && gy < N && gy >= row_lo && gy < row_hi &&
                                   (gy >> 1) >= win.emit_lo && (gy >> 1) < win.emit_hi;
                T n[W], s2[W];
#pragma unroll
                for (int e = 0; e < W; ++e) {
                    n[e] = (i == 0) ? rup[e] : res[i - 1][e];
                    s2[e] = (i == RW - 1) ? rdn[e] : res[i + 1][e];
                }
                const T nl = from_left(n[W - 1]), sl = from_left(s2[W - 1]), cl = from_left(res[i][W - 1]);
#pragma unroll
                for (int e = 0; e < W; e += 2) {
                    const T c = res[i][e];
                    T corners = (e == 0 ? nl : n[e - 1]) + n[e + 1];
                    corners = corners + (e == 0 ? sl : s2[e - 1]);
                    corners = corners + s2[e + 1];
                    T edges = (e == 0 ? cl : res[i][e - 1]) + res[i][e + 1];
                    edges = edges + n[e];
                    edges = edges + s2[e];
                    const T o = wgt * ((corners + (T)2 * edges) + (T)4 * c);
                    const int J = (gx0 + e) >> 1;
                    if (rowst && colout && J >= 1 && J < NC) {
                        const long at = (long)(gy >> 1) * cpitch + J;
                        coarse_b[at] = o;
                        if (coarse_zero) coarse_zero[at] = (T)0;
                    }
                }
            }
        }
    }
    MGX_PHASE_END(kPhaseTile, N | (PRE << 16) | (POST << 20) | (RW << 24));
}

static __global__ void __launch_bounds__(kBlock)
k_axpy_f32_to_f64(double* __restrict__ u, const float* __restrict__ e, double scale, int N, long pitch, long epitch,
                  int row_lo, int row_hi, int R, int strips, int chunks, int assign)
{
    const Tile t = wave_tile(strips, chunks);
    if (!t.active) return;
    const Cols c = lane_cols<2>(t.strip, N, pitch);
    const int r0 = row_lo + t.chunk * R;
    const int r1 = min(r0 + R, row_hi);
    for (int r = r0; r < r1; ++r) {
        if (c.st) {
            const float2 ev = *reinterpret_cast<const float2*>(e + (long)r * epitch + c.col);
            double2* pu = reinterpret_cast<double2*>(u + (long)r * pitch + c.col);
            double2 o = assign ? make_double2(0.0, 0.0) : *pu;
            o.x = o.x + scale * (double)ev.x;
            o.y = o.y + scale * (double)ev.y;
            if (c.col == 0) o.x = 0.0;
            *pu = o;
        }
    }
}

static __global__ void __launch_bounds__(kBlock)
k_update_residual(const double* __restrict__ u, const float* __restrict__ e, const double* __restrict__ rhs,
                  double* __restrict__ unew, float* __restrict__ r32, double scale, double inv_scale,
                  double* __restrict__ partial, int N, long pitch, long epitch, int row_lo, int row_hi,
                  int R, int strips, int chunks)
{
    __shared__ double wsum[kWavesPerBlock];
    const Tile t = wave_tile(strips, chunks);
    double acc = 0.0;
    if (t.active) {
        const Cols c = lane_cols<2>(t.strip, N, pitch);
        const int r0 = row_lo + t.chunk * R;
        const int r1 = min(r0 + R, row_hi);
        auto updated = [&](int r) {
            double2 o = make_double2(0.0, 0.0);
            if (c.ld) {
                const double2 uv = *reinterpret_cast<const double2*>(u + (long)r * pitch + c.col);
                const float2 ev = *reinterpret_cast<const float2*>(e + (long)r * epitch + c.col);
                o.x = uv.x + scale * (double)ev.x;
                o.y = uv.y + scale * (double)ev.y;
                if (c.col == 0) o.x = 0.0;
            }
            return o;
        };
        double2 up = updated(r0 - 1);
        double2 cur = updated(r0);
        for (int r = r0; r < r1; ++r) {
            const double2 dn = updated(r + 1);
            const double2 bb = vload<double2>(rhs + (long)r * pitch + c.col, c.ld);
            double2 o = residual_vec(up, cur, dn, bb);
            mask_cols(o, c.col, N);
            if (c.st) {
                *reinterpret_cast<double2*>(unew + (long)r * pitch + c.col) = cur;
                acc += (double)o.x * (double)o.x + (double)o.y * (double)o.y;
                *reinterpret_cast<float2*>(r32 + (long)r * epitch + c.col) =
                    make_float2((float)(o.x * inv_scale), (float)(o.y * inv_scale));
            }
            up = cur; cur = dn;
        }
    }
    for (int off = 32; off > 0; off >>= 1) acc += __shfl_down(acc, off, kWave);
    if ((threadIdx.x & 63) == 0) wsum[threadIdx.x >> 6] = acc;
    __syncthreads();
    if (threadIdx.x == 0) {
        double s = 0.0;
        for (int w = 0; w < kWavesPerBlock; ++w) s += wsum[w];
        partial[blockIdx.x] = s;
    }
}

static __global__ void __launch_bounds__(kBlock)
k_scale_f64_to_f32(float* __restrict__ out, const double* __restrict__ in, double inv_scale, int N, long pitch_in, long pitch_out,
                   int row_lo, int row_hi, int R, int strips, int chunks)
{
    const Tile t = wave_tile(strips, chunks);
    if (!t.active) return;
    const Cols c = lane_cols<2>(t.strip, N, pitch_in);
    const int r0 = row_lo + t.chunk * R;
    const int r1 = min(r0 + R, row_hi);
    for (int r = r0; r < r1; ++r) {
        if (c.st) {
            double2 x = *reinterpret_cast<const double2*>(in + (long)r * pitch_in + c.col);
            if (c.col == 0) x.x = 0.0;
            *reinterpret_cast<float2*>(out + (long)r * pitch_out + c.col) =
                make_float2((float)(x.x * inv_scale), (float)(x.y * inv_scale));
        }
    }
}

struct Launch { int R, strips, chunks, blocks; };

inline Launch make_launch(int N, int W, int rows, int rows_per_chunk)
{
    Launch L;
    const int nvec_out = N / W;
    L.strips = (nvec_out + kOutLanes - 1) / kOutLanes;
    if (L.strips < 1) L.strips = 1;
    int R = rows_per_chunk;
    if (R <= 0) {
        R = rows / 128;
        if (R < 4) R = 4;
        if (R > 8) R = 8;
    }
    L.R = R;
    L.chunks = (rows + R - 1) / R;
    if (L.chunks < 1) L.chunks = 1;
    const long waves = (long)L.strips * L.chunks;
    long blocks = (waves + kWavesPerBlock - 1) / kWavesPerBlock;
    blocks = (blocks + 7) / 8 * 8;
    L.blocks = (int)blocks;
    return L;
}

}
```

multigrid_nikhil_c-_amd/csrc/mgx_launch.hpp:

```cpp
#pragma once

#include "../../include/mgx.h"
#include "mgx_kernels.hpp"
#include "mgx_pass_plan.hpp"

#include <algorithm>

namespace mgx {

inline long level_pitch(int level, int dtype)
{
    const long N = 1L << level;
    const long align = (dtype == MGX_DTYPE_F64) ? 32 : 64;
    return (N + 1 + align - 1) / align * align;
}

template <typename T> struct JacobiCoef { T c0, c1; };
template <typename T>
JacobiCoef<T> jacobi_coef(double omega)
{
    const T om = (T)omega;
    return {(T)(1.0 - (double)om), (T)((double)om / 4.0)};
}

// ... 72 lines not shown
            default: break;
        }
    }
    return false;
}

struct FoldArgs {
    const void* coarse_e = nullptr;
    void* coarse_b = nullptr;
    void* coarse_zero = nullptr;
    int restrict_mode = 0;
    double* partial = nullptr;
    long cpitch = 0;
    int zero_in = 0;
    int row_lo = 0, row_hi = 0;
    CycleWin win{0, 0, 0, 0, 0, 0};
};

inline GeomKnobs geom_knobs()
{
    GeomKnobs k;
    k.edge_short = env_int("MGX_EDGE_SHORT", 1) != 0;
    k.edge_pct = env_int("MGX_EDGE_PCT", 23);
    k.last_pct = env_int("MGX_LAST_PCT", 38);
    k.min_chunk = std::max(8, env_int("MGX_MIN_CHUNK", 16));
    k.min_rounds = std::max(1, env_int("MGX_MIN_ROUNDS", 1));
    k.min_rounds_rows = env_int("MGX_MIN_ROUNDS_ROWS", 1024);
    k.pair = env_int("MGX_PAIR", 1) != 0;
    k.pair_ratio = std::max(100, env_int("MGX_PAIR_RATIO", 130));
    k.pair_max_rows = env_int("MGX_PAIR_MAX_ROWS", 640);
    k.pair_min_rows = env_int("MGX_PAIR_MIN_ROWS", 150);
    return k;
}
template <typename T, int K, int PRE, int POST, int SM, int AR>
int launch_cycle_k(const T* vin, const T* b, T* vout, const FoldArgs& fa, int N, long pitch, T c0, T c1, int R,
                   hipStream_t st)
{
    constexpr int OUT = cycle_out_lanes<K, POST, VecOf<T>::W>();
    constexpr bool BL = cycle_b_in_lds<T, K, POST, SM>();
    constexpr int E = (POST == 1 ? 3 : (POST == 2 ? 2 : 0)) + (cycle_skew<T, K, PRE, POST, SM, AR>() > 0 ? 1 : 0);
    constexpr int kTripSteps = BL ? kBRing : trip_steps<T>();
    const int row_lo = fa.row_lo, row_hi = fa.row_hi;
    const CycleWin& win = fa.win;
    if (POST == 1 && !(row_lo & 1)) return -1;
    const int strips = (N / VecOf<T>::W + OUT - 1) / OUT;
    const bool auto_rows = R < 0;
    if (auto_rows) R = -R;
    constexpr int ETOP = POST ? 1 : 0, EBOT = POST == 1 ? 2 : (POST == 2 ? 1 : 0);
    const bool top_edge = (row_lo - K - ETOP) < std::max(win.row_first, 1) || (PRE && ((row_lo - K - ETOP) >> 1) < win.crow_first);
    const bool bot_edge = (row_hi + K + EBOT - 1) > std::min(win.row_last, N - 1) || (PRE && ((row_hi + K + EBOT) >> 1) > win.crow_last);
    GeomKnobs kn = BL ? geom_knobs() : GeomKnobs();
    if (sizeof(T) == 4 && BL) kn.pair_min_rows = std::min(kn.pair_min_rows, env_int("MGX_PAIR_MIN_ROWS_F32", 100));
    const CycleGeom g = cycle_geom_pick(row_lo, row_hi, strips, 2 * K + E, kTripSteps, R, auto_rows, BL, kn, top_edge, bot_edge);
    const int blocks = g.blocks;
    const T w = (fa.restrict_mode == MGX_RESTRICT_FW16) ? (T)0.0625 : (T)0.25;
    hipLaunchKernelGGL((k_jacobi_cycle<T, K, PRE, POST, SM, AR>), dim3(blocks), dim3(kBlock), 0, st, vin, b, vout,
                       (const T*)fa.coarse_e, (T*)fa.coarse_b, (T*)fa.coarse_zero, w, fa.partial, N, pitch, fa.cpitch,
                       row_lo, row_hi, g.R, strips, g.chunks, g.Re, g.chunks_e, g.row_last0, g.Rl, g.RB, g.n_tall, g.n_short, g.Rf, c0, c1, fa.zero_in, win);
    return blocks;
}

template <typename T, int PRE, int POST, int SM, int AR>
int launch_cycle(int K, const T* vin, const T* b, T* vout, const FoldArgs& fa, int N, long pitch, T c0, T c1, int R,
                 hipStream_t st)
{
    switch (K) {
        case 2: return launch_cycle_k<T, 2, PRE, POST, SM, AR>(vin, b, vout, fa, N, pitch, c0, c1, R, st);
        case 4: return launch_cycle_k<T, 4, PRE, POST, SM, AR>(vin, b, vout, fa, N, pitch, c0, c1, R, st);
        case 6: return launch_cycle_k<T, 6, PRE, POST, SM, AR>(vin, b, vout, fa, N, pitch, c0, c1, R, st);
        default: break;
    }
    if constexpr (sizeof(T) == 8 || PRE == 1 || POST == 0) {
        if (K == 8) return launch_cycle_k<T, 8, PRE, POST, SM, AR>(vin, b, vout, fa, N, pitch, c0, c1, R, st);
    }
    if constexpr (!(PRE == 1 && POST == 1) && !(SM == 1 && POST == 1) && !(sizeof(T) == 4 && PRE == 1 && POST == 2) &&
                  !(sizeof(T) == 4 && POST == 1 && AR == 0)) {
        if (K == 10) return launch_cycle_k<T, 10, PRE, POST, SM, AR>(vin, b, vout, fa, N, pitch, c0, c1, R, st);
    }
    if constexpr (SM == 0) {
        switch (K) {
            case 1: return launch_cycle_k<T, 1, PRE, POST, 0, AR>(vin, b, vout, fa, N, pitch, c0, c1, R, st);
            case 3: return launch_cycle_k<T, 3, PRE, POST, 0, AR>(vin, b, vout, fa, N, pitch, c0, c1, R, st);
            case 5: return launch_cycle_k<T, 5, PRE, POST, 0, AR>(vin, b, vout, fa, N, pitch, c0, c1, R, st);
            default: break;
        }
    }
    return -1;
}

template <int PRE_, int POST_> struct Stages { static constexpr int PRE = PRE_, POST = POST_; };
template <typename F>
int with_stages(bool pre, int post, F&& f)
{
    if (pre) return post == 2 ? f(Stages<1, 2>{}) : (post == 1 ? f(Stages<1, 1>{}) : f(Stages<1, 0>{}));
    return post == 2 ? f(Stages<0, 2>{}) : (post == 1 ? f(Stages<0, 1>{}) : f(Stages<0, 0>{}));
}

template <typename T, int SM, int PRE, int POST, int AR>
int launch_tile(const T* vin, const T* b, T* vout, const FoldArgs& fa, int N, long pitch, T c0, T c1, int levels,
                hipStream_t st)
{
    const int He = levels + tile_extra<POST>();
    const int TH = kTileSY - 2 * He, TW = kTileSX - 2 * He;
    if (TH < 8 || TW < 8) return -1;
    const int row_lo = fa.row_lo, row_hi = fa.row_hi;
    const CycleWin& win = fa.win;
    const int tiles_y = (row_hi - row_lo + TH - 1) / TH, tiles_x = (N - 1 + TW - 1) / TW;
    if (tiles_y < 1) return 0;
    const T w = (fa.restrict_mode == MGX_RESTRICT_FW16) ? (T)0.0625 : (T)0.25;
    hipLaunchKernelGGL((k_tile_smooth<T, SM, PRE, POST, AR>), dim3(tiles_y * tiles_x), dim3(kBlock), 0, st, vin, b, vout,
                       (const T*)fa.coarse_e, (T*)fa.coarse_b, (T*)fa.coarse_zero, w, fa.partial, N, pitch, fa.cpitch,
                       levels, c0, c1, tiles_x, fa.zero_in, row_lo, row_hi, win);
    return tiles_y * tiles_x;
}

template <typename T, int SM, int PRE, int POST, int AR>
int launch_tile_wide(const T* vin, const T* b, T* vout, const FoldArgs& fa, int N, long pitch, T c0, T c1, int levels,
                     int rw, hipStream_t st)
{
    if (VecOf<T>::W == 4) rw = 8;
    const int row_lo = fa.row_lo, row_hi = fa.row_hi;
    const CycleWin& win = fa.win;
    const TileWideGeom g = tile_wide_geom(N, row_lo, row_hi, levels + tile_extra<POST>(), VecOf<T>::W, rw);
    if (g.TH < 8 || g.TW < 8) return -1;
    if (g.tiles_y < 1) return 0;
    const T w = (fa.restrict_mode == MGX_RESTRICT_FW16) ? (T)0.0625 : (T)0.25;
    const dim3 grid(g.tiles_y * g.tiles_x), block(kTileWideWaves * kWave);
    if (rw == 8)
        hipLaunchKernelGGL((k_tile_wide<T, SM, PRE, POST, AR, 8>), grid, block, 0, st, vin, b, vout, (const T*)fa.coarse_e,
                           (T*)fa.coarse_b, (T*)fa.coarse_zero, w, fa.partial, N, pitch, fa.cpitch, levels, c0, c1, g.tiles_x,
                           fa.zero_in, row_lo, row_hi, win);
    else if constexpr (VecOf<T>::W == 2) {
        if (rw != 10) return -1;
        hipLaunchKernelGGL((k_tile_wide<T, SM, PRE, POST, AR, 10>), grid, block, 0, st, vin, b, vout, (const T*)fa.coarse_e,
                           (T*)fa.coarse_b, (T*)fa.coarse_zero, w, fa.partial, N, pitch, fa.cpitch, levels, c0, c1, g.tiles_x,
                           fa.zero_in, row_lo, row_hi, win);
    } else {
        return -1;
    }
    return g.tiles_y * g.tiles_x;
}

template <typename T, int SM, int AR>
int launch_tile_pass(const T* vin, const T* b, T* vout, const FoldArgs& fa, int N, long pitch, T c0, T c1, int levels,
                     int band, bool pre, int post, hipStream_t st)
{
    return with_stages(pre, post, [&](auto s) {
        using S = decltype(s);
        return band ? launch_tile_wide<T, SM, S::PRE, S::POST, AR>(vin, b, vout, fa, N, pitch, c0, c1, levels, band, st)
                    : launch_tile<T, SM, S::PRE, S::POST, AR>(vin, b, vout, fa, N, pitch, c0, c1, levels, st);
    });
}

template <typename T>
void launch_restrict(const T* v, const T* b, T* cb, T* czero, int N, long pitch, long cpitch,
                     int crow_lo, int crow_hi, int fine_row_off, int mode, bool fused, int rpc, hipStream_t st)
{
    if (crow_hi <= crow_lo) return;
    Launch g = make_launch(N, VecOf<T>::W, crow_hi - crow_lo, rpc > 0 ? (rpc + 1) / 2 : 0);
    const T w = (mode == MGX_RESTRICT_FW16) ? (T)0.0625 : (T)0.25;
    if (fused)
        hipLaunchKernelGGL((k_restrict<T, true>), dim3(g.blocks), dim3(kBlock), 0, st, v, b, cb, czero, N, pitch,
                           cpitch, crow_lo, crow_hi, fine_row_off, g.R, g.strips, g.chunks, w);
    else
        hipLaunchKernelGGL((k_restrict<T, false>), dim3(g.blocks), dim3(kBlock), 0, st, v, b, cb, czero, N, pitch,
                           cpitch, crow_lo, crow_hi, fine_row_off, g.R, g.strips, g.chunks, w);
}

template <typename T>
void launch_prolong(T* v, const T* e, int N, long pitch, long cpitch, int row_lo, int row_hi,
                    int fine_row_off, bool add, int rpc, hipStream_t st)
{
    if (row_hi <= row_lo) return;
    const Launch g = make_launch(N, VecOf<T>::W, row_hi - row_lo, rpc);
    if (add)
        hipLaunchKernelGGL((k_prolong<T, true>), dim3(g.blocks), dim3(kBlock), 0, st, v, e, N, pitch, cpitch,
                           row_lo, row_hi, fine_row_off, g.R, g.strips, g.chunks);
    else
        hipLaunchKernelGGL((k_prolong<T, false>), dim3(g.blocks), dim3(kBlock), 0, st, v, e, N, pitch, cpitch,
                           row_lo, row_hi, fine_row_off, g.R, g.strips, g.chunks);
}

template <typename T> long sumsq_blocks(int N, int rows, int rpc)
{
    return make_launch(N, VecOf<T>::W, rows, rpc).blocks;
}

template <typename T, int MODE>
void launch_residual(const T* v, const T* b, void* out, long pitch_out, double* partial, double* sum_dev,
                     double inv_scale, int N, long pitch, int row_lo, int row_hi, int rpc, hipStream_t st,
                     long partial_cap, int rows_alloc)
{
    Launch g = make_launch(N, VecOf<T>::W, row_hi - row_lo, rpc);
    if (MODE != 0 && partial_cap >= 0 && g.blocks > partial_cap) {
        const int R = (int)(((long)g.strips * (row_hi - row_lo) / kWavesPerBlock + partial_cap - 9) / (partial_cap - 8)) + 1;
        g = make_launch(N, VecOf<T>::W, row_hi - row_lo, R);
    }
    hipLaunchKernelGGL((k_residual<T, MODE>), dim3(g.blocks), dim3(kBlock), 0, st, v, b, out, pitch_out, partial,
                       inv_scale, N, pitch, row_lo, row_hi, g.R, g.strips, g.chunks, rows_alloc);
    if (MODE != 0)
        hipLaunchKernelGGL(k_reduce_partials, dim3(1), dim3(kReduceThreads), 0, st, partial, g.blocks, sum_dev);
}


#define MGX_FOR_SMAR(X, T) X(T, 0, 0) X(T, 0, 1) X(T, 1, 0)
#define MGX_DECL_CYCLE_PP(T, PRE, POST, SM, AR) \
    extern template int launch_cycle<T, PRE, POST, SM, AR>(int, const T*, const T*, T*, const FoldArgs&, int, long, T, T, int, hipStream_t);
#define MGX_DECL_CYCLE(T, SM, AR) MGX_DECL_CYCLE_PP(T, 1, 2, SM, AR) MGX_DECL_CYCLE_PP(T, 1, 0, SM, AR) MGX_DECL_CYCLE_PP(T, 0, 1, SM, AR) \
    MGX_DECL_CYCLE_PP(T, 0, 2, SM, AR) MGX_DECL_CYCLE_PP(T, 1, 1, SM, AR)
#define MGX_DECL_FUSED(T, SM, AR) \
    extern template bool launch_fused<T, SM, AR>(int, const T*, const T*, T*, int, long, int, int, T, T, int, int, int, int, hipStream_t, int, int);
#define MGX_DECL_TILE(T, SM, AR) \
    extern template int launch_tile_pass<T, SM, AR>(const T*, const T*, T*, const FoldArgs&, int, long, T, T, int, int, bool, int, hipStream_t);
#if !defined(MGX_INST_KIND) && !defined(MGX_SINGLE_TU)
MGX_FOR_SMAR(MGX_DECL_CYCLE, double) MGX_FOR_SMAR(MGX_DECL_CYCLE, float)
MGX_FOR_SMAR(MGX_DECL_FUSED, double) MGX_FOR_SMAR(MGX_DECL_FUSED, float)
MGX_FOR_SMAR(MGX_DECL_TILE, double) MGX_FOR_SMAR(MGX_DECL_TILE, float)
#endif

}
```

multigrid_nikhil_c-_amd/csrc/mgx_pass_plan.hpp:

```cpp
#pragma once

#include "../../include/mgx.h"
#include "mgx_geom.hpp"

#include <algorithm>
#include <cstdlib>
#include <vector>

namespace mgx {

inline int env_int(const char* name, int dflt)
{
    const char* s = getenv(name);
    return (s && *s) ? atoi(s) : dflt;
}

struct FuseCfg {
    int kmax; int rows; int min_n; int fold_kmax; int fold_kmax_big; int tile_max_n; int tile_k; int fold_kmax_nopost;
    int tile_wide; int tile_short_n;
    int plan_pre[8] = {0}; int n_pre = 0; int plan_post[8] = {0}; int n_post = 0; int plan_min_n = 8192;
    int arith = 0;
};

inline int fuse_rows_deep(int N, int rows)
{
    const int strips = (N / 2 + 51) / 52;
    const int cpr = std::max(1, 2048 / strips);
    for (int m = 1; m <= 64; ++m) {
        const int R = (rows + m * cpr - 1) / (m * cpr);
        if (R <= 200) return std::max(R, 16);
    }
    return 64;
}

inline bool fuse_rows_auto(const FuseCfg& fc, int N, int K, bool f64)
{
    return fc.rows <= 0 && K >= (f64 ? 8 : 10) && N >= 2048;
}

inline int shallow_big_n() { static const int n = env_int("MGX_SHALLOW_BIG_N", 8192); return n; }
inline int shallow_mid_rows() { static const int r = env_int("MGX_SHALLOW_ROWS_MID", 48); return r; }

inline int fuse_rows(const FuseCfg& fc, int N, int K, bool f64 = true, int rows = 0)
{
    if (fc.rows > 0) return fc.rows;
    if (K <= 2) {
        static const int big2 = env_int("MGX_SHALLOW2_ROWS_BIG", 96);
        return N >= shallow_big_n() ? big2 : (N >= 4096 ? shallow_mid_rows() : 8);
    }
    if (K <= 4) {
        static const int big = env_int("MGX_SHALLOW_ROWS_BIG", 96);
        return N >= shallow_big_n() ? big : (N >= 4096 ? shallow_mid_rows() : 16);
    }
    if (f64 && K >= 8 && N >= 2048) return fuse_rows_deep(N, rows > 0 ? rows : N - 1);
    int R = N / 128;
    if (R < 8) R = 8;
    if (R > (f64 ? 64 : 32)) R = f64 ? 64 : 32;
    return R;
}

inline FuseCfg fuse_cfg()
{
    FuseCfg f;
    f.kmax = env_int("MGX_FUSE", 10);
    if (f.kmax < 1) f.kmax = 1;
    if (f.kmax > 10) f.kmax = 10;
    f.rows = env_int("MGX_FUSE_ROWS", 0);
    if (f.rows < 0) f.rows = 0;
    f.min_n = std::max(64, env_int("MGX_FUSE_MIN_N", 256));
    f.fold_kmax = std::max(1, std::min(f.kmax, env_int("MGX_FOLD_KMAX", 10)));
    f.fold_kmax_big = std::max(1, std::min(f.kmax, env_int("MGX_FOLD_KMAX_BIG", 10)));
    f.tile_wide = std::max(0, std::min(2, env_int("MGX_TILE_WIDE", 1)));
    f.tile_short_n = env_int("MGX_TILE_SHORT_N", 512);
    f.tile_max_n = std::max(0, env_int("MGX_TILE_MAX_N", 1024));
    f.tile_k = std::max(2, std::min(10, env_int("MGX_TILE_K", 10)));
    f.fold_kmax_nopost = std::max(1, std::min(f.kmax, env_int("MGX_FOLD_KMAX_NOPOST", 10)));
    auto parse = [](const char* name, int* out) {
        const char* v = std::getenv(name);
        int n = 0;
        while (v && *v && n < 8) {
            char* end = nullptr;
            const long k = std::strtol(v, &end, 10);
            if (end == v || k < 1 || k > 10) return 0;
            out[n++] = (int)k;
            v = (*end == ',') ? end + 1 : end;
            if (*end && *end != ',') return 0;
        }
        return n;
    };
    f.n_pre = parse("MGX_PLAN_PRE", f.plan_pre);
    f.n_post = parse("MGX_PLAN_POST", f.plan_post);
    f.plan_min_n = env_int("MGX_PLAN_MIN_N", 8192);
    return f;
}

inline bool cycle_k_supported(int K, bool rbgs, bool f64, int post, bool pre, int arith)
{
    if (K == 10) return !(pre && post == 1) && !(rbgs && post == 1) && !(!f64 && pre && post == 2) && !(!f64 && post == 1 && arith == 0);
    if (K == 8 && !f64 && !pre && post != 0) return false;
    return rbgs ? (K == 2 || K == 4 || K == 6 || K == 8) : (K >= 1 && K <= 8 && K != 7);
}

inline bool fused_k_supported(int K, bool rbgs)
{
    return K == 2 || K == 4 || K == 6 || K == 8 || K == 10 || (!rbgs && (K == 3 || K == 5));
}

inline int tile_band(const FuseCfg& fc, int N, bool f64)
{
    return (fc.tile_wide >= (f64 ? 1 : 2)) ? tile_wide_rw(N, fc.tile_short_n) : 0;
}

constexpr double kFuseRate64[11] = {0, 1.00, 1.80, 2.45, 3.16, 3.81, 4.80, 0, 5.60, 0, 5.63};
constexpr double kFuseRate32[11] = {0, 1.00, 1.67, 2.38, 3.10, 3.77, 4.26, 0, 4.98, 0, 4.67};
constexpr double kFuseRateGS64[11] = {0, 1.00, 1.81, 2.50, 3.19, 3.12, 0, 0, 0, 0, 0};
constexpr double kFuseRateGS32[11] = {0, 1.00, 1.79, 2.20, 2.87, 2.69, 0, 0, 0, 0, 0};

inline double fold_pass_cost(int K, bool rbgs, int post, bool f64, int arith)
{
    if (!cycle_k_supported(K, rbgs, f64, post, false, arith)) return -1.0;
    if (rbgs) return K <= 4 ? 1.0 : (K == 6 ? 1.1 : (K == 8 ? 1.3 : 2.4));
    if (K <= 5) return 1.0;
    if (!f64) return K == 6 ? 1.34 : (K == 8 ? 1.53 : 1.75);
    if (K == 6) return 1.05;
    if (K == 8) return 1.12;
    return 1.46;
}

template <typename Cost>
std::vector<int> split_sweeps(int mu, int smax, double launch, double eps, Cost cost)
{
    std::vector<double> best(mu + 1, 1e300);
    std::vector<int> pick(mu + 1, 1);
    best[0] = 0.0;
    for (int m = 1; m <= mu; ++m)
        for (int k = 1; k <= std::min(m, smax); ++k) {
            const double c = cost(k, m);
            if (c < 0.0) continue;
            const double t = best[m - k] + c + launch;
            if (t < best[m] - eps) { best[m] = t; pick[m] = k; }
        }
    std::vector<int> parts;
    for (int m = mu; m > 0; m -= pick[m]) parts.push_back(pick[m]);
    return parts;
}

enum PassKind {
    PASS_JACOBI,
    PASS_RBGS,
    PASS_FUSED,
    PASS_FOLDED,
    PASS_TILE,
};

struct Pass {
    int kind;
    int K;
    bool pre; int post;
    bool zero_in;
    int lo, hi;
    int R;
};

struct BlockReq {
    int smoother = MGX_SMOOTHER_JACOBI; bool f64 = true;
    int N = 0, row0 = 0, rows = 0;
    int row_lo = 0, row_hi = 0;
    int mu = 0;
    bool pre = false;
    int post = 0;
    bool zero_in = false;
    bool widen = true;
    bool strict = false;
    long tile_points = 0;
    int rpc = 0;
};

inline bool fold_plan(const FuseCfg& fc, const BlockReq& q, std::vector<Pass>* plan)
{
    plan->clear();
    const bool rbgs = (q.smoother == MGX_SMOOTHER_RBGS);
    const int per = rbgs ? 2 : 1, N = q.N, mu = q.mu;
    const int first = 1 - q.row0, last = N - q.row0;
    {
        const int lo = std::max(std::max(q.row_lo, first), 1), hi = std::min(std::min(q.row_hi, last), q.rows - 1);
        const bool whole = q.row_lo <= first && q.row_hi >= last;
        if (fc.tile_max_n > 0 && hi > lo && (long)(hi - lo) * N <= q.tile_points && (per * mu <= fc.tile_k || whole)) {
            const int smax = std::max(1, fc.tile_k / per), np = (mu + smax - 1) / smax;
            for (int p = 0; p < np; ++p) {
                const int sw = mu / np + (p < mu % np ? 1 : 0);
                plan->push_back({PASS_TILE, per * sw, q.pre && p == 0, p == np - 1 ? q.post : 0, q.zero_in && p == 0,
                                 lo + q.row0, hi + q.row0, tile_band(fc, N, q.f64)});
            }
            return true;
        }
    }
    const bool staged = q.pre || q.post != 0;
    const bool fuse = fc.kmax > per && N >= fc.min_n && (q.row_hi - q.row_lo) >= 64 && mu <= 64;
    std::vector<int> parts;
    if (!staged) {
        const double* rate = rbgs ? (q.f64 ? kFuseRateGS64 : kFuseRateGS32) : (q.f64 ? kFuseRate64 : kFuseRate32);
        if (fuse)
            parts = split_sweeps(mu, std::max(1, std::min(fc.kmax, 10) / per), 0.02, 0.0,
                                 [&](int k, int) { return rate[k] > 0.0 ? (double)k / rate[k] : -1.0; });
        else
            parts.assign(std::max(mu, 0), 1);
    } else {
        const int* forced = nullptr;
        int nf = 0;
        if (!q.pre && q.post == 1) { forced = fc.plan_pre; nf = fc.n_pre; }
        else if (q.pre) { forced = fc.plan_post; nf = fc.n_post; }
        if (nf > 0 && N >= fc.plan_min_n) {
            int sum = 0;
            bool ok = true;
            for (int i = 0; i < nf; ++i) {
                sum += forced[i];
                const int K = per * forced[i];
                const bool folded = (i == 0 && q.pre) || (i == nf - 1 && q.post != 0);
                const int Q = (i == nf - 1) ? q.post : 0;
                ok = ok && K <= 10 && (folded ? cycle_k_supported(K, rbgs, q.f64, Q, q.pre && i == 0, fc.arith) : (K != 7 && K != 9 && (!rbgs || K % 2 == 0)));
            }
            if (ok && sum == mu) parts.assign(forced, forced + nf);
        }
        if (parts.empty()) {
            int kcap = N >= 8192 ? fc.fold_kmax_big : fc.fold_kmax;
            if (q.post == 0) kcap = std::min(kcap, fc.fold_kmax_nopost);
            if (rbgs) kcap = std::min(kcap, env_int("MGX_FOLD_KMAX_GS", 10));
            if (q.pre && q.post == 1) kcap = std::min(kcap, 8);
            parts = split_sweeps(mu, std::max(1, kcap / per), 1e-3, 1e-12, [&](int k, int m) {
                if (k == mu && m == mu && !cycle_k_supported(per * k, rbgs, q.f64, q.post, q.pre, fc.arith)) return -1.0;
                return fold_pass_cost(per * k, rbgs, q.post, q.f64, fc.arith);
            });
            std::sort(parts.begin(), parts.end(), [](int a, int b) { return a > b; });
        }
    }
    const int np = (int)parts.size();
    const int stage_rows = q.post == 2 ? 1 : (q.post == 1 ? 2 : 0);
    int done = 0;
    for (int p = 0; p < np; ++p) {
        const int sw = parts[p], K = per * sw;
        const bool P = q.pre && p == 0, zin = q.zero_in && p == 0;
        const int Q = (p == np - 1) ? q.post : 0;
        const int ext = q.widen ? per * (mu - (done + sw)) + (p != np - 1 ? stage_rows : 0) : 0;
        int lo = std::max(q.row_lo - ext, first), hi = std::min(q.row_hi + ext, last);
        if (q.strict && hi > lo && (std::max(lo - K, first - 1) < 0 || std::min(hi + K - 1, last) > q.rows - 1)) return false;
        lo = std::max(lo, 1);
        hi = std::min(hi, q.rows - 1);
        const int kind = (P || Q) ? PASS_FOLDED : (!rbgs && K == 1) ? PASS_JACOBI : (rbgs && !staged && !fuse) ? PASS_RBGS : PASS_FUSED;
        int R = q.rpc;
        if (kind == PASS_FUSED || kind == PASS_FOLDED) R = fuse_rows(fc, N, K, q.f64, hi - lo);
        if (hi > lo) {
            if (kind == PASS_FOLDED) {
                if (!cycle_k_supported(K, rbgs, q.f64, Q, P, fc.arith)) return false;
                if (Q == 1 && !((lo + q.row0) & 1)) return false;
                if (fuse_rows_auto(fc, N, K, q.f64)) R = -R;
            }
            if (kind == PASS_FUSED && !fused_k_supported(K, rbgs)) return false;
            if (zin && (kind == PASS_JACOBI || kind == PASS_RBGS)) return false;
        }
        plan->push_back({kind, K, P, Q, zin, lo + q.row0, hi + q.row0, R});
        done += sw;
    }
    return true;
}

}
```

multigrid_nikhil_c-_amd/csrc/mgx_phase_trace.hpp:

```cpp
#pragma once

#include <hip/hip_runtime.h>

#ifdef MGX_WAVE_TRACE
namespace mgx {

constexpr int kPhaseMax = 24;
constexpr int kPhaseCap = 1 << 14;
constexpr int kPhaseDst = 0, kPhaseTile = 1;
struct PhaseTrace { int kind, tag, block, n; long long t[kPhaseMax]; };
__device__ PhaseTrace g_phase_trace[kPhaseCap];
__device__ unsigned g_phase_trace_n;

__device__ __forceinline__ void phase_mark(long long* t, int& n)
{
    if (threadIdx.x < 64) {
        const long long c = wall_clock64();
        if (threadIdx.x == 0 && n < kPhaseMax) t[n] = c;
    }
    ++n;
}
template <typename X> __device__ __forceinline__ void phase_mark_after(long long* t, int& n, const X& v)
{
    asm volatile("" ::"v"(v) : "memory");
    phase_mark(t, n);
}
__device__ __forceinline__ void phase_flush(const long long* t, int n, int kind, int tag)
{
    if (threadIdx.x == 0) {
        PhaseTrace& r = g_phase_trace[atomicAdd(&g_phase_trace_n, 1u) & (kPhaseCap - 1)];
        r.kind = kind; r.tag = tag; r.block = (int)blockIdx.x; r.n = n < kPhaseMax ? n : kPhaseMax;
        for (int q = 0; q < r.n; ++q) r.t[q] = t[q];
    }
}

}
#define MGX_PHASE_BEGIN() __shared__ long long ph_t[mgx::kPhaseMax]; int ph_n = 0; mgx::phase_mark(ph_t, ph_n)
#define MGX_PHASE() mgx::phase_mark(ph_t, ph_n)
#define MGX_PHASE_AFTER(v) mgx::phase_mark_after(ph_t, ph_n, (v))
#define MGX_PHASE_END(kind, tag) (mgx::phase_mark(ph_t, ph_n), mgx::phase_flush(ph_t, ph_n, (kind), (tag)))
#else
#define MGX_PHASE_BEGIN() ((void)0)
#define MGX_PHASE() ((void)0)
#define MGX_PHASE_AFTER(v) ((void)0)
#define MGX_PHASE_END(kind, tag) ((void)0)
#endif
```

Measured before the change: 1164 billion.

## Fuse multiple V-cycle ascent levels into one tiled prolong-and-smooth kernel

Adds a k_tile_up kernel that performs the upward leg of the V-cycle for up to three levels at once. Each block corrects and smooths a coarse tile with halo, hands it to the next finer level through shared memory, and finishes with the fine-level smoothing. The intermediate coarse-level post-smooth results are only partially computed, so those levels are marked stale and lazily recomputed (settle_up) before any API reads them. The aim is to cut kernel launches and global memory round trips per level on the ascent. The cost is redundant halo computation, higher register and shared memory pressure, and more complex state tracking, including graph-capture bookkeeping.

```diff
diff --git a/multigrid_nikhil_c-_amd/csrc/mgx.hip b/multigrid_nikhil_c-_amd/csrc/mgx.hip
--- a/multigrid_nikhil_c-_amd/csrc/mgx.hip
+++ b/multigrid_nikhil_c-_amd/csrc/mgx.hip
@@ -87,10 +87,12 @@
     int use_zero_in = 1;
     int norm_blocks_ready = 0;
     double fine_updates = 0.0;
+    unsigned up_stale = 0;
     struct CycleGraph {
         std::vector<void*> before, after;
         hipGraphExec_t exec = nullptr;
         double fine_updates = 0.0;
+        unsigned up_stale = 0;
     };
     std::vector<CycleGraph> graphs;
     int use_graph = 1;
@@ -900,6 +902,7 @@
 bool descend(mgx_solver* s, int level, bool zero_in_here, const MultiSet& a = kOwnSet, double* fu = nullptr)
 {
     const bool zin_next = own(a) && zero_in_ok(s, level - 1);
+    if (own(a)) s->up_stale &= ~(1u << (level - 1));
     if (!own(a) || !smooth_folded(s, level, s->cfg.mu1, false, 1, zero_in_here, zin_next)) {
         if (zero_in_here) (void)zero_u(s, level, a);
         smooth(s, level, s->cfg.mu1, false, a, fu);
@@ -916,8 +919,71 @@
     }
 }
 
+int up_fuse_depth_at(const mgx_solver* s, int level, int post, int kind, const MultiSet& a)
+{
+    if (!own(a) || kind != MGX_CYCLE_V || s->cycle != MGX_CYCLE_V || s->var || s->mixed || s->fuse.up_fuse < 2) return 1;
+    std::vector<Pass> plans[kTileUpMaxDepth];
+    int n = 0;
+    for (; n < kTileUpMaxDepth && level - n > s->cfg.coarsest_level; ++n) {
+        const Level& l = s->lv[level - n];
+        const int q = n == 0 ? post : 0;
+        if (!l.f64 || !tile_level(s, l) || !fold_eligible(s, l, s->cfg.mu2, true, q)) break;
+        if (!fold_plan(s->fuse, level_req(s, l, s->cfg.mu2, true, q, false, 0), &plans[n])) break;
+    }
+    return n < 2 ? 1 : up_fuse_depth(s->fuse, plans, n, s->lv[level].N);
+}
+
+void settle_up(mgx_solver* s)
+{
+    for (int l = s->cfg.coarsest_level + 1; l < s->cfg.finest_level && s->up_stale; ++l) {
+        if (!((s->up_stale >> l) & 1u)) continue;
+        s->up_stale &= ~(1u << l);
+        std::swap(s->lv[l].u, s->lv[l].tmp);
+        (void)smooth_folded(s, l, s->cfg.mu2, true, 0);
+    }
+}
+
+void ascend_fused(mgx_solver* s, int level, int depth, int post)
+{
+    Level& l = s->lv[level];
+    const bool fine = (level == s->cfg.finest_level);
+    const int mu = s->cfg.mu2;
+    std::vector<Pass> plan;
+    int nb = -1;
+    if (fold_plan(s->fuse, level_req(s, l, mu, true, post, false, 0), &plan) && up_fuse_stage(plan, l.N, true)) {
+        Prof p(s, fine ? MGX_PROF_SMOOTH_FINE : MGX_PROF_COARSE, 1);
+        nb = with_kernel_set(true, s->cfg.smoother, s->fuse.arith, [&](auto k) {
+            using K = decltype(k);
+            using T = typename K::T;
+            TileUpArgs<T> ua{};
+            for (int q = 0; q < depth; ++q) {
+                const Level& lq = s->lv[level - q];
+                ua.vin[q] = (const T*)lq.u; ua.rhs[q] = (const T*)lq.b; ua.pitch[q] = lq.pitch;
+            }
+            ua.coarse_e = (const T*)s->lv[level - depth].u; ua.cpitch = s->lv[level - depth].pitch;
+            ua.vout = (T*)l.tmp; ua.partial = s->partial;
+            const JacobiCoef<T> jc = jacobi_coef<T>(s->cfg.omega);
+            return launch_tile_up<T, K::SM, K::AR>(ua, l.N, jc.c0, jc.c1, plan[0].K, plan[0].R, depth, post, s->stream);
+        });
+        p.set(1, (long long)mu * (fine ? 1 : depth));
+    }
+    if (fine && nb >= 0) { Prof pc(s, MGX_PROF_COARSE, 0); pc.set(0, (long long)mu * (depth - 1)); }
+    for (int q = 1; q < depth; ++q) {
+        s->up_stale |= 1u << (level - q);
+        std::swap(s->lv[level - q].u, s->lv[level - q].tmp);
+    }
+    if (nb < 0) {
+        settle_up(s);
+        ascend(s, level, post, kOwnSet, nullptr);
+        return;
+    }
+    std::swap(l.u, l.tmp);
+    if (post == 2) s->norm_blocks_ready = nb;
+    if (fine) s->fine_updates += (double)mu * (double)(l.N - 1) * (double)(l.N - 1);
+}
+
 void vcycle(mgx_solver* s, int level, bool zero_in_here = false, int post_top = 0, int kind = -1, const MultiSet& a = kOwnSet,
-            double* fu = nullptr);
+            double* fu = nullptr, int absorb = 0);
 
 bool small_level(const mgx_solver* s, int level, const MultiSet& a)
 {
@@ -953,7 +1019,7 @@
     p.set(1, (ascend ? s->cfg.mu2 : 0) + (descend ? s->cfg.mu1 : 0));
 }
 
-void coarse_visits(mgx_solver* s, int level, bool zero_in_here, int kind, const MultiSet& a = kOwnSet, double* fu = nullptr)
+void coarse_visits(mgx_solver* s, int level, bool zero_in_here, int kind, const MultiSet& a = kOwnSet, double* fu = nullptr, int absorb = 0)
 {
     const bool twice = kind != MGX_CYCLE_V && level > s->cfg.coarsest_level;
     const int second = kind == MGX_CYCLE_F ? MGX_CYCLE_V : kind;
@@ -965,11 +1031,11 @@
         small_visit(s, level, true, false);
         return;
     }
-    vcycle(s, level, zero_in_here, 0, kind, a, fu);
+    vcycle(s, level, zero_in_here, 0, kind, a, fu, absorb);
     if (twice) vcycle(s, level, false, 0, second, a, fu);
 }
 
-void vcycle(mgx_solver* s, int level, bool zero_in_here, int post_top, int kind, const MultiSet& a, double* fu)
+void vcycle(mgx_solver* s, int level, bool zero_in_here, int post_top, int kind, const MultiSet& a, double* fu, int absorb)
 {
     if (kind < 0) kind = s->cycle;
     if (level == s->cfg.coarsest_level) {
@@ -988,13 +1054,17 @@
         return;
     }
     const bool zin_next = descend(s, level, zero_in_here, a, fu);
-    coarse_visits(s, level - 1, zin_next, kind, a, fu);
-    ascend(s, level, post_top, a, fu);
+    const int depth = absorb > 0 ? absorb : up_fuse_depth_at(s, level, post_top, kind, a);
+    coarse_visits(s, level - 1, zin_next, kind, a, fu, depth - 1);
+    if (absorb > 0) return;
+    if (depth > 1) ascend_fused(s, level, depth, post_top);
+    else ascend(s, level, post_top, a, fu);
 }
 
 int fmg(mgx_solver* s)
 {
     const int lo = s->cfg.coarsest_level, hi = s->cfg.finest_level;
+    settle_up(s);
     for (int l = hi; l > lo; --l) restrict_level(s, l, false, false);
     if (s->cfg.bottom == MGX_BOTTOM_EXACT) {
         bottom_solve(s);
@@ -1058,10 +1128,12 @@
         if (c.before == key) {
             set_buffer_state(s, c.after);
             s->fine_updates += c.fine_updates;
+            s->up_stale = c.up_stale;
             return c.exec;
         }
     if (s->graphs.size() >= kMaxGraphs) return nullptr;
     const double fu0 = s->fine_updates;
+    const unsigned stale0 = s->up_stale;
     hipGraph_t graph = nullptr;
     hipGraphExec_t exec = nullptr;
     hipError_t e = hipStreamBeginCapture(s->stream, hipStreamCaptureModeThreadLocal);
@@ -1078,10 +1150,11 @@
         (void)hipGetLastError();
         set_buffer_state(s, key);
         s->fine_updates = fu0;
+        s->up_stale = stale0;
         s->use_graph = 0;
         return nullptr;
     }
-    s->graphs.push_back({key, buffer_state(s), exec, s->fine_updates - fu0});
+    s->graphs.push_back({key, buffer_state(s), exec, s->fine_updates - fu0, s->up_stale});
     return exec;
 }
 
@@ -1171,6 +1244,7 @@
 
 Level* pick(mgx_solver* s, int level, int which, void** grid)
 {
+    if (level < s->cfg.finest_level) settle_up(s);
     Level* l = &s->lv[level];
     if (s->mixed && level == s->cfg.finest_level) l = &s->fine64;
     switch (which) {
@@ -1846,7 +1920,8 @@
     if (level < (lvl_min) || level > s->cfg.finest_level)                                 \
         return s->fail(MGX_ERR_INVALID, "level out of range for this operator");          \
     MIXED_GUARD(level)                                                                    \
-    if (int vr__ = var_ready(s, s->cfg.coarsest_level, level)) return vr__;
+    if (int vr__ = var_ready(s, s->cfg.coarsest_level, level)) return vr__;               \
+    settle_up(s);
 
 #define OP_EPILOGUE                                                                       \
     HIPCHK(s, hipGetLastError());                                                         \
@@ -1906,6 +1981,7 @@
     if (s->cfg.bottom != MGX_BOTTOM_EXACT) return s->fail(MGX_ERR_STATE, "handle was created with bottom = SMOOTH");
     MIXED_GUARD(s->cfg.coarsest_level)
     if (int vr = var_ready(s, s->cfg.coarsest_level, s->cfg.coarsest_level)) return vr;
+    settle_up(s);
     bottom_solve(s);
     OP_EPILOGUE
 }
diff --git a/multigrid_nikhil_c-_amd/csrc/mgx_geom.hpp b/multigrid_nikhil_c-_amd/csrc/mgx_geom.hpp
--- a/multigrid_nikhil_c-_amd/csrc/mgx_geom.hpp
+++ b/multigrid_nikhil_c-_amd/csrc/mgx_geom.hpp
@@ -25,6 +25,7 @@
 struct CTile { int strip, r0, r1; bool active; };
 
 MGX_GEOM_HD int geom_min(int a, int b) { return a < b ? a : b; }
+MGX_GEOM_HD int geom_max(int a, int b) { return a > b ? a : b; }
 
 MGX_GEOM_HD CTile cycle_tile_at(int block, int wave, int grid, int strips, int chunks, int chunks_e, int R, int Re, int row_lo,
                                 int row_hi, int row_last0, int Rl, int RB, int n_tall, int n_short, int Rf)
@@ -273,4 +274,42 @@
 
 MGX_GEOM_HD int tile_wide_rw(int N, int short_max_n) { return N <= short_max_n ? 8 : 10; }
 
-}
+constexpr int kTileUpMaxDepth = 3;
+constexpr int kTileUpHalo = 10;
+
+struct TileUpStage {
+    int oy, ox;
+    int y0, y1, x0, x1;
+};
+
+MGX_GEOM_HD constexpr int tile_up_rows(int rw_top, int k, int He)
+{
+    return k == 0 ? kTileWideWaves * rw_top : (tile_up_rows(rw_top, k - 1, He) + 1) / 2 + 1 + 2 * He;
+}
+MGX_GEOM_HD constexpr int tile_up_rw(int rw_top, int k)
+{
+    return k == 0 ? rw_top : (tile_up_rows(rw_top, k, kTileUpHalo) + kTileWideWaves - 1) / kTileWideWaves;
+}
+MGX_GEOM_HD constexpr bool tile_up_fits(int rw_top, int depth, int He)
+{
+    if (depth < 1 || depth > kTileUpMaxDepth || He < 1) return false;
+    for (int k = 1; k < depth; ++k)
+        if (tile_up_rows(rw_top, k, He) > kTileWideWaves * tile_up_rw(rw_top, k)) return false;
+    return true;
+}
+
+MGX_GEOM_HD TileUpStage tile_up_below(int fy0, int fy1, int fx0, int fx1, int NC, int He)
+{
+    TileUpStage s;
+    s.y0 = geom_max(fy0 >> 1, 0); s.y1 = geom_min((fy1 + 1) >> 1, NC);
+    s.x0 = geom_max(fx0 >> 1, 0); s.x1 = geom_min((fx1 + 1) >> 1, NC);
+    s.oy = s.y0 - He;
+    s.ox = (s.x0 - He) & ~1;
+    return s;
+}
+MGX_GEOM_HD TileUpStage tile_up_below(const TileUpStage& f, int NC, int He)
+{
+    return tile_up_below(f.y0 - He, f.y1 + He, f.x0 - He, f.x1 + He, NC, He);
+}
+
+}
diff --git a/multigrid_nikhil_c-_amd/csrc/mgx_inst.hip b/multigrid_nikhil_c-_amd/csrc/mgx_inst.hip
--- a/multigrid_nikhil_c-_amd/csrc/mgx_inst.hip
+++ b/multigrid_nikhil_c-_amd/csrc/mgx_inst.hip
@@ -64,7 +64,9 @@
 #elif MGX_INST_KIND == 12
 template void launch_eig_project_dots<T_>(int, int, const T_* const*, const T_* const*, double*, double*, const EigGeom&, hipStream_t);
 template void launch_eig_project_sub<T_>(int, int, const T_* const*, T_* const*, const double*, const EigGeom&, hipStream_t);
+#elif MGX_INST_KIND == 13
+template int launch_tile_up<T_, MGX_INST_SM, MGX_INST_AR>(const TileUpArgs<T_>&, int, T_, T_, int, int, int, int, hipStream_t);
 #else
-#error "MGX_INST_KIND must be 1 .. 12"
+#error "MGX_INST_KIND must be 1 .. 13"
 #endif
 }
diff --git a/multigrid_nikhil_c-_amd/csrc/mgx_kernels.hpp b/multigrid_nikhil_c-_amd/csrc/mgx_kernels.hpp
--- a/multigrid_nikhil_c-_amd/csrc/mgx_kernels.hpp
+++ b/multigrid_nikhil_c-_amd/csrc/mgx_kernels.hpp
@@ -1593,111 +1593,124 @@
 __device__ __forceinline__ double2 vmake(const double (&a)[2]) { return make_double2(a[0], a[1]); }
 __device__ __forceinline__ float4 vmake(const float (&a)[4]) { return make_float4(a[0], a[1], a[2], a[3]); }
 
-template <typename T, int SM, int PRE, int POST, int AR, int RW>
-__global__ void __launch_bounds__(kTileWideWaves * kWave)
-k_tile_wide(const T* __restrict__ vin, const T* __restrict__ rhs, T* __restrict__ vout,
-            const T* __restrict__ coarse_e, T* __restrict__ coarse_b, T* __restrict__ coarse_zero, T wgt,
-            double* __restrict__ partial, int N, long pitch, long cpitch, int levels, T c0, T c1,
-            int tiles_x, int zero_in, int row_lo, int row_hi, CycleWin win)
+template <typename T> struct TileLane {
+    int gx0;
+    bool vld;
+    bool cu[VecOf<T>::W];
+};
+template <typename T>
+__device__ __forceinline__ TileLane<T> tile_lane(int gx0, int N)
+{
+    TileLane<T> ln;
+    ln.gx0 = gx0;
+    ln.vld = gx0 >= 0 && gx0 < N;
+    const bool cu0 = ln.vld && gx0 > 0;
+#pragma unroll
+    for (int e = 0; e < VecOf<T>::W; ++e) ln.cu[e] = e == 0 ? cu0 : ln.vld;
+    return ln;
+}
+
+template <int RW> constexpr int tile_ncr() { return (RW + 1) / 2 + 1; }
+
+template <typename T, int RW>
+__device__ __forceinline__ unsigned tile_load(const T* __restrict__ vin, const T* __restrict__ rhs, int N, long pitch, int gy0,
+                                              const TileLane<T>& ln, int zero_in, const CycleWin& win,
+                                              T (&u)[RW][VecOf<T>::W], T (&b)[RW][VecOf<T>::W])
 {
     using V = typename VecOf<T>::type;
     constexpr int W = VecOf<T>::W;
-    constexpr int NW = kTileWideWaves;
-    __shared__ V edge[2][NW][2][kWave];
-    __shared__ double wsum[NW];
-    MGX_PHASE_BEGIN();
-    const TileWideGeom g = tile_wide_geom(N, row_lo, row_hi, levels + tile_extra<POST>(), W, RW);
-    const int He = g.He, TH = g.TH, TW = g.TW;
-    const int lane = threadIdx.x & 63;
-    const int wv = __builtin_amdgcn_readfirstlane(threadIdx.x >> 6);
-    const int ty = blockIdx.x / tiles_x, tx = blockIdx.x - ty * tiles_x;
-    const int y0 = wv * RW;
-    const int gy0 = row_lo + ty * TH - He + y0;
-    const int cx0 = tx * TW;
-    const int gx0 = cx0 - g.Hx + W * lane;
-    const bool vld = gx0 >= 0 && gx0 < N;
-    const bool cu0 = vld && gx0 > 0;
-    bool cu[W];
-#pragma unroll
-    for (int e = 0; e < W; ++e) cu[e] = e == 0 ? cu0 : vld;
-    const int NC = N / 2;
-    MGX_PHASE_AFTER(gx0 + gy0);
-
-    T u[RW][W], b[RW][W];
     unsigned rowmask = 0;
 #pragma unroll
     for (int i = 0; i < RW; ++i) {
         const int gy = gy0 + i;
         const bool rowok = gy > 0 && gy < N && gy >= win.row_first && gy <= win.row_last;
         if (rowok) rowmask |= 1u << i;
-        const long at = (long)gy * pitch + gx0;
+        const long at = (long)gy * pitch + ln.gx0;
         V uv = vzero((V*)nullptr), bv = vzero((V*)nullptr);
-        if (vld && rowok) {
+        if (ln.vld && rowok) {
             bv = *reinterpret_cast<const V*>(rhs + at);
             if (!zero_in) uv = *reinterpret_cast<const V*>(vin + at);
         }
 #pragma unroll
         for (int e = 0; e < W; ++e) {
-            u[i][e] = cu[e] ? vget(uv, e) : (T)0;
-            b[i][e] = cu[e] ? vget(bv, e) : (T)0;
-        }
-    }
-    if (PRE) {
-        constexpr int NCR = RW / 2 + 1, NCC = W / 2 + 1;
-        const int kc0 = gy0 >> 1, J = gx0 >> 1;
-        T cr[NCR][NCC];
-#pragma unroll
-        for (int k = 0; k < NCR; ++k) {
-            const int cy = kc0 + k;
-            const bool ok = vld && cy >= 0 && cy <= NC && cy >= win.crow_first && cy <= win.crow_last;
-            const T* ep = coarse_e + (long)cy * cpitch + J;
-#pragma unroll
-            for (int m = 0; m < NCC; ++m) cr[k][m] = ok ? ep[m] : (T)0;
-        }
-        auto correct = [&](auto parity) {
-            constexpr int par = decltype(parity)::value;
-#pragma unroll
-            for (int i = 0; i < RW; ++i) {
-                const int gy = gy0 + i;
-                const bool rodd = ((par + i) & 1) != 0;
-                const int kr = (par + i) >> 1;
-                const bool rin = ((rowmask >> i) & 1u) && (gy >> 1) >= win.crow_first && (gy >> 1) + (rodd ? 1 : 0) <= win.crow_last;
-#pragma unroll
-                for (int e = 0; e < W; ++e) {
-                    const bool codd = (e & 1) != 0;
-                    const bool unk = cu[e] && rin;
-                    const T a00 = unk ? cr[kr][e >> 1] : (T)0;
-                    const T a01 = (unk && codd) ? cr[kr][(e >> 1) + 1] : (T)0;
-                    const T a10 = (unk && rodd) ? cr[kr + (rodd ? 1 : 0)][e >> 1] : (T)0;
-                    const T a11 = (unk && rodd && codd) ? cr[kr + (rodd ? 1 : 0)][(e >> 1) + 1] : (T)0;
-                    const T ev = codd ? (T)0.5 * (a00 + a01) : a00;
-                    const T od = codd ? (T)0.25 * (((a00 + a10) + a01) + a11) : (T)0.5 * (a00 + a10);
-                    const T add = rodd ? od : ev;
-                    u[i][e] = unk ? u[i][e] + add : u[i][e];
-                }
+            u[i][e] = ln.cu[e] ? vget(uv, e) : (T)0;
+            b[i][e] = ln.cu[e] ? vget(bv, e) : (T)0;
+        }
+    }
+    return rowmask;
+}
+
+template <typename T, int RW, typename Fetch>
+__device__ __forceinline__ void tile_coarse(int gy0, const TileLane<T>& ln, int NC, const CycleWin& win, Fetch&& fetch,
+                                            T (&cr)[tile_ncr<RW>()][VecOf<T>::W / 2 + 1])
+{
+    const int kc0 = gy0 >> 1, J = ln.gx0 >> 1;
+#pragma unroll
+    for (int k = 0; k < tile_ncr<RW>(); ++k) {
+        const int cy = kc0 + k;
+        const bool ok = ln.vld && cy >= 0 && cy <= NC && cy >= win.crow_first && cy <= win.crow_last;
+#pragma unroll
+        for (int m = 0; m < VecOf<T>::W / 2 + 1; ++m) cr[k][m] = ok ? fetch(cy, J + m) : (T)0;
+    }
+}
+
+template <typename T, int RW>
+__device__ __forceinline__ void tile_correct(int gy0, const TileLane<T>& ln, unsigned rowmask, const CycleWin& win,
+                                             const T (&cr)[tile_ncr<RW>()][VecOf<T>::W / 2 + 1], T (&u)[RW][VecOf<T>::W])
+{
+    constexpr int W = VecOf<T>::W;
+    auto correct = [&](auto parity) {
+        constexpr int par = decltype(parity)::value;
+#pragma unroll
+        for (int i = 0; i < RW; ++i) {
+            const int gy = gy0 + i;
+            const bool rodd = ((par + i) & 1) != 0;
+            const int kr = (par + i) >> 1;
+            const bool rin = ((rowmask >> i) & 1u) && (gy >> 1) >= win.crow_first && (gy >> 1) + (rodd ? 1 : 0) <= win.crow_last;
+#pragma unroll
+            for (int e = 0; e < W; ++e) {
+                const bool codd = (e & 1) != 0;
+                const bool unk = ln.cu[e] && rin;
+                const T a00 = unk ? cr[kr][e >> 1] : (T)0;
+                const T a01 = (unk && codd) ? cr[kr][(e >> 1) + 1] : (T)0;
+                const T a10 = (unk && rodd) ? cr[kr + (rodd ? 1 : 0)][e >> 1] : (T)0;
+                const T a11 = (unk && rodd && codd) ? cr[kr + (rodd ? 1 : 0)][(e >> 1) + 1] : (T)0;
+                const T ev = codd ? (T)0.5 * (a00 + a01) : a00;
+                const T od = codd ? (T)0.25 * (((a00 + a10) + a01) + a11) : (T)0.5 * (a00 + a10);
+                const T add = rodd ? od : ev;
+                u[i][e] = unk ? u[i][e] + add : u[i][e];
             }
-        };
-        if (gy0 & 1) correct(std::integral_constant<int, 1>{});
-        else correct(std::integral_constant<int, 0>{});
-    }
-
-    MGX_PHASE_AFTER(b[RW - 1][W - 1]);
-    MGX_PHASE_AFTER(u[RW - 1][W - 1]);
-
-    int buf = 0;
-    auto halo_rows = [&](const T (&a)[RW][W], T (&up)[W], T (&dn)[W]) {
-        edge[buf][wv][0][lane] = vmake(a[0]);
-        edge[buf][wv][1][lane] = vmake(a[RW - 1]);
-        __syncthreads();
-        const V uv = wv > 0 ? edge[buf][wv - 1][1][lane] : vzero((V*)nullptr);
-        const V dv = wv < NW - 1 ? edge[buf][wv + 1][0][lane] : vzero((V*)nullptr);
-#pragma unroll
-        for (int e = 0; e < W; ++e) { up[e] = vget(uv, e); dn[e] = vget(dv, e); }
-        buf ^= 1;
+        }
     };
+    if (gy0 & 1) correct(std::integral_constant<int, 1>{});
+    else correct(std::integral_constant<int, 0>{});
+}
+
+template <typename T, int RW>
+__device__ __forceinline__ void tile_halo_rows(typename VecOf<T>::type (&edge)[2][kTileWideWaves][2][kWave], int& buf, int wv, int lane,
+                                               const T (&a)[RW][VecOf<T>::W], T (&up)[VecOf<T>::W], T (&dn)[VecOf<T>::W])
+{
+    using V = typename VecOf<T>::type;
+    edge[buf][wv][0][lane] = vmake(a[0]);
+    edge[buf][wv][1][lane] = vmake(a[RW - 1]);
+    __syncthreads();
+    const V uv = wv > 0 ? edge[buf][wv - 1][1][lane] : vzero((V*)nullptr);
+    const V dv = wv < kTileWideWaves - 1 ? edge[buf][wv + 1][0][lane] : vzero((V*)nullptr);
+#pragma unroll
+    for (int e = 0; e < VecOf<T>::W; ++e) { up[e] = vget(uv, e); dn[e] = vget(dv, e); }
+    buf ^= 1;
+}
+
+template <typename T, int SM, int AR, int RW>
+__device__ __forceinline__ void tile_sweeps(typename VecOf<T>::type (&edge)[2][kTileWideWaves][2][kWave], int& buf, int wv, int lane, int levels,
+                                            T c0, T c1, int gy0, const TileLane<T>& ln, unsigned rowmask,
+                                            T (&u)[RW][VecOf<T>::W], const T (&b)[RW][VecOf<T>::W], PhaseRef ph)
+{
+    constexpr int W = VecOf<T>::W;
+    MGX_PHASE_USE(ph);
     for (int j = 1; j <= levels; ++j) {
         T up[W], dn[W];
-        halo_rows(u, up, dn);
+        tile_halo_rows<T, RW>(edge, buf, wv, lane, u, up, dn);
         const int colour = (j - 1) & 1;
         T prev[W];
 #pragma unroll
@@ -1715,10 +1728,10 @@
                 const T we = e == 0 ? l : cur[e - 1], ea = e == W - 1 ? r : cur[e + 1];
                 if (SM == 0) {
                     const T o = jac_pt<AR>(c0, cur[e], c1 * b[i][e], c1, nbr(prev[e], we, ea, below));
-                    u[i][e] = (cu[e] && rowact) ? o : cur[e];
+                    u[i][e] = (ln.cu[e] && rowact) ? o : cur[e];
                 } else {
                     const T o = (T)0.25 * (b[i][e] + nbr(prev[e], we, ea, below));
-                    u[i][e] = (cu[e] && rowact && ((gy0 + i + e) & 1) == colour) ? o : cur[e];
+                    u[i][e] = (ln.cu[e] && rowact && ((gy0 + i + e) & 1) == colour) ? o : cur[e];
                 }
             }
 #pragma unroll
@@ -1726,7 +1739,21 @@
         }
         MGX_PHASE_AFTER(u[RW - 1][W - 1]);
     }
-
+}
+
+template <typename T, int POST, int RW>
+__device__ __forceinline__ void tile_finish(typename VecOf<T>::type (&edge)[2][kTileWideWaves][2][kWave], int& buf, double (&wsum)[kTileWideWaves],
+                                            int wv, int lane, T* __restrict__ vout, T* __restrict__ coarse_b, T* __restrict__ coarse_zero,
+                                            T wgt, double* __restrict__ partial, int N, long pitch, long cpitch, int row_lo, int row_hi,
+                                            const CycleWin& win, const TileWideGeom& g, int y0, int gy0, int cx0, const TileLane<T>& ln,
+                                            const T (&u)[RW][VecOf<T>::W], const T (&b)[RW][VecOf<T>::W], PhaseRef ph)
+{
+    using V = typename VecOf<T>::type;
+    constexpr int W = VecOf<T>::W;
+    constexpr int NW = kTileWideWaves;
+    MGX_PHASE_USE(ph);
+    const int He = g.He, TH = g.TH, TW = g.TW, NC = N / 2, gx0 = ln.gx0;
+    const bool (&cu)[W] = ln.cu;
     const bool colout = gx0 >= cx0 && gx0 < cx0 + TW && gx0 < N;
 #pragma unroll
     for (int i = 0; i < RW; ++i) {
@@ -1738,7 +1765,7 @@
 
     if (POST != 0) {
         T up[W], dn[W];
-        halo_rows(u, up, dn);
+        tile_halo_rows<T, RW>(edge, buf, wv, lane, u, up, dn);
         T res[RW][W];
         double acc = 0.0;
         T prev[W];
@@ -1776,7 +1803,7 @@
         }
         if (POST == 1) {
             T rup[W], rdn[W];
-            halo_rows(res, rup, rdn);
+            tile_halo_rows<T, RW>(edge, buf, wv, lane, res, rup, rdn);
 #pragma unroll
             for (int i = 0; i < RW; ++i) {
                 const int y = y0 + i, gy = gy0 + i;
@@ -1809,7 +1836,144 @@
             }
         }
     }
+}
+
+template <typename T, int SM, int PRE, int POST, int AR, int RW>
+__global__ void __launch_bounds__(kTileWideWaves * kWave)
+k_tile_wide(const T* __restrict__ vin, const T* __restrict__ rhs, T* __restrict__ vout,
+            const T* __restrict__ coarse_e, T* __restrict__ coarse_b, T* __restrict__ coarse_zero, T wgt,
+            double* __restrict__ partial, int N, long pitch, long cpitch, int levels, T c0, T c1,
+            int tiles_x, int zero_in, int row_lo, int row_hi, CycleWin win)
+{
+    using V = typename VecOf<T>::type;
+    constexpr int W = VecOf<T>::W;
+    constexpr int NW = kTileWideWaves;
+    __shared__ V edge[2][NW][2][kWave];
+    __shared__ double wsum[NW];
+    MGX_PHASE_BEGIN();
+    const TileWideGeom g = tile_wide_geom(N, row_lo, row_hi, levels + tile_extra<POST>(), W, RW);
+    const int lane = threadIdx.x & 63;
+    const int wv = __builtin_amdgcn_readfirstlane(threadIdx.x >> 6);
+    const int ty = blockIdx.x / tiles_x, tx = blockIdx.x - ty * tiles_x;
+    const int y0 = wv * RW;
+    const int gy0 = row_lo + ty * g.TH - g.He + y0;
+    const int cx0 = tx * g.TW;
+    const TileLane<T> ln = tile_lane<T>(cx0 - g.Hx + W * lane, N);
+    MGX_PHASE_AFTER(ln.gx0 + gy0);
+
+    T u[RW][W], b[RW][W];
+    const unsigned rowmask = tile_load<T, RW>(vin, rhs, N, pitch, gy0, ln, zero_in, win, u, b);
+    if (PRE) {
+        T cr[tile_ncr<RW>()][W / 2 + 1];
+        tile_coarse<T, RW>(gy0, ln, N / 2, win, [&](int cy, int cx) { return coarse_e[(long)cy * cpitch + cx]; }, cr);
+        tile_correct<T, RW>(gy0, ln, rowmask, win, cr, u);
+    }
+    MGX_PHASE_AFTER(b[RW - 1][W - 1]);
+    MGX_PHASE_AFTER(u[RW - 1][W - 1]);
+
+    int buf = 0;
+    tile_sweeps<T, SM, AR, RW>(edge, buf, wv, lane, levels, c0, c1, gy0, ln, rowmask, u, b, MGX_PHASE_REF());
+    tile_finish<T, POST, RW>(edge, buf, wsum, wv, lane, vout, coarse_b, coarse_zero, wgt, partial, N, pitch, cpitch, row_lo, row_hi,
+                             win, g, y0, gy0, cx0, ln, u, b, MGX_PHASE_REF());
     MGX_PHASE_END(kPhaseTile, N | (PRE << 16) | (POST << 20) | (RW << 24));
+}
+
+template <typename T> struct TileUpArgs {
+    const T* vin[kTileUpMaxDepth];
+    const T* rhs[kTileUpMaxDepth];
+    long pitch[kTileUpMaxDepth];
+    const T* coarse_e; long cpitch;
+    T* vout;
+    double* partial;
+};
+
+template <typename T, int RW, int HP>
+__device__ __forceinline__ void tile_hand_over(T* hand, const TileUpStage& st, int gy0, const TileLane<T>& ln, const T (&u)[RW][VecOf<T>::W])
+{
+#pragma unroll
+    for (int i = 0; i < RW; ++i) {
+        const int gy = gy0 + i;
+        const bool rowin = gy >= st.y0 && gy <= st.y1;
+#pragma unroll
+        for (int e = 0; e < VecOf<T>::W; ++e) {
+            const int gx = ln.gx0 + e;
+            if (rowin && gx >= st.x0 && gx <= st.x1) hand[(gy - st.y0) * HP + (gx - st.x0)] = u[i][e];
+        }
+    }
+}
+
+template <typename T, int SM, int AR, int RW, int DEPTH, int POST>
+__global__ void __launch_bounds__(kTileWideWaves * kWave)
+k_tile_up(TileUpArgs<T> a, int N, int levels, T c0, T c1, int tiles_x)
+{
+    using V = typename VecOf<T>::type;
+    constexpr int W = VecOf<T>::W;
+    constexpr int NW = kTileWideWaves;
+    static_assert(W == 2 && (DEPTH == 2 || DEPTH == 3) && (POST == 0 || POST == 2), "fp64 tiles, two or three stages, no restriction");
+    constexpr int RW1 = tile_up_rw(RW, 1), RW2 = tile_up_rw(RW, 2);
+    constexpr int RWL = DEPTH == 3 ? RW2 : RW1;
+    constexpr int HR = NW * RW / 2 + 1, HP = kWave * W / 2 + 2;
+    __shared__ V edge[2][NW][2][kWave];
+    __shared__ double wsum[NW];
+    __shared__ T hand[HR * HP];
+    MGX_PHASE_BEGIN();
+    const int row_lo = 1, row_hi = N;
+    const TileWideGeom g = tile_wide_geom(N, row_lo, row_hi, levels + tile_extra<POST>(), W, RW);
+    const int lane = threadIdx.x & 63;
+    const int wv = __builtin_amdgcn_readfirstlane(threadIdx.x >> 6);
+    const int ty = blockIdx.x / tiles_x, tx = blockIdx.x - ty * tiles_x;
+    const int ay0 = row_lo + ty * g.TH - g.He;
+    const int cx0 = tx * g.TW, ax0 = cx0 - g.Hx;
+    const int N1 = N / 2, N2 = N / 4;
+    const TileUpStage s1 = tile_up_below(ay0, ay0 + NW * RW - 1, ax0, ax0 + kWave * W - 1, N1, levels);
+    const TileUpStage s2 = tile_up_below(s1, N2, levels);
+    const CycleWin win0{0, N, 0, N1, 0, 0}, win1{0, N1, 0, N2, 0, 0}, win2{0, N2, 0, N2 / 2, 0, 0};
+    const int y0 = wv * RW;
+    const int gy0 = ay0 + y0, gy1 = s1.oy + wv * RW1, gy2 = s2.oy + wv * RW2;
+    const TileLane<T> ln0 = tile_lane<T>(ax0 + W * lane, N), ln1 = tile_lane<T>(s1.ox + W * lane, N1), ln2 = tile_lane<T>(s2.ox + W * lane, N2);
+    MGX_PHASE_AFTER(ln0.gx0 + gy0);
+
+    T u0[RW][W], b0[RW][W], u1[RW1][W], b1[RW1][W], u2[RW2][W], b2[RW2][W];
+    T crl[tile_ncr<RWL>()][W / 2 + 1];
+    unsigned rowmask2 = 0;
+    auto from_memory = [&](int cy, int cx) { return a.coarse_e[(long)cy * a.cpitch + cx]; };
+    if constexpr (DEPTH == 3) {
+        rowmask2 = tile_load<T, RW2>(a.vin[2], a.rhs[2], N2, a.pitch[2], gy2, ln2, 0, win2, u2, b2);
+        tile_coarse<T, RW2>(gy2, ln2, N2 / 2, win2, from_memory, crl);
+    }
+    const unsigned rowmask1 = tile_load<T, RW1>(a.vin[1], a.rhs[1], N1, a.pitch[1], gy1, ln1, 0, win1, u1, b1);
+    if constexpr (DEPTH == 2) tile_coarse<T, RW1>(gy1, ln1, N1 / 2, win1, from_memory, crl);
+    unsigned rowmask0 = 0;
+    if constexpr (DEPTH == 2) rowmask0 = tile_load<T, RW>(a.vin[0], a.rhs[0], N, a.pitch[0], gy0, ln0, 0, win0, u0, b0);
+
+    int buf = 0;
+    auto from_hand = [&](const TileUpStage& st) {
+        return [&](int cy, int cx) {
+            return (cy >= st.y0 && cy <= st.y1 && cx >= st.x0 && cx <= st.x1) ? hand[(cy - st.y0) * HP + (cx - st.x0)] : (T)0;
+        };
+    };
+    if constexpr (DEPTH == 3) {
+        tile_correct<T, RW2>(gy2, ln2, rowmask2, win2, crl, u2);
+        tile_sweeps<T, SM, AR, RW2>(edge, buf, wv, lane, levels, c0, c1, gy2, ln2, rowmask2, u2, b2, MGX_PHASE_REF());
+        tile_hand_over<T, RW2, HP>(hand, s2, gy2, ln2, u2);
+        rowmask0 = tile_load<T, RW>(a.vin[0], a.rhs[0], N, a.pitch[0], gy0, ln0, 0, win0, u0, b0);
+        __syncthreads();
+        T cr1[tile_ncr<RW1>()][W / 2 + 1];
+        tile_coarse<T, RW1>(gy1, ln1, N1 / 2, win1, from_hand(s2), cr1);
+        tile_correct<T, RW1>(gy1, ln1, rowmask1, win1, cr1, u1);
+    } else {
+        tile_correct<T, RW1>(gy1, ln1, rowmask1, win1, crl, u1);
+    }
+    tile_sweeps<T, SM, AR, RW1>(edge, buf, wv, lane, levels, c0, c1, gy1, ln1, rowmask1, u1, b1, MGX_PHASE_REF());
+    tile_hand_over<T, RW1, HP>(hand, s1, gy1, ln1, u1);
+    __syncthreads();
+    T cr0[tile_ncr<RW>()][W / 2 + 1];
+    tile_coarse<T, RW>(gy0, ln0, N1, win0, from_hand(s1), cr0);
+    tile_correct<T, RW>(gy0, ln0, rowmask0, win0, cr0, u0);
+    tile_sweeps<T, SM, AR, RW>(edge, buf, wv, lane, levels, c0, c1, gy0, ln0, rowmask0, u0, b0, MGX_PHASE_REF());
+    tile_finish<T, POST, RW>(edge, buf, wsum, wv, lane, a.vout, (T*)nullptr, (T*)nullptr, (T)0, a.partial, N, a.pitch[0], a.cpitch, row_lo, row_hi,
+                             win0, g, y0, gy0, cx0, ln0, u0, b0, MGX_PHASE_REF());
+    MGX_PHASE_END(kPhaseTile, N | (1 << 16) | (POST << 20) | (RW << 24));
 }
 
 static __global__ void __launch_bounds__(kBlock)
diff --git a/multigrid_nikhil_c-_amd/csrc/mgx_launch.hpp b/multigrid_nikhil_c-_amd/csrc/mgx_launch.hpp
--- a/multigrid_nikhil_c-_amd/csrc/mgx_launch.hpp
+++ b/multigrid_nikhil_c-_amd/csrc/mgx_launch.hpp
@@ -248,6 +248,32 @@
     });
 }
 
+template <typename T, int SM, int AR>
+int launch_tile_up(const TileUpArgs<T>& a, int N, T c0, T c1, int levels, int rw, int depth, int post, hipStream_t st)
+{
+    if constexpr (VecOf<T>::W == 2) {
+        const int He = levels + (post == 2 ? tile_extra<2>() : 0);
+        const TileWideGeom g = tile_wide_geom(N, 1, N, He, VecOf<T>::W, rw);
+        if ((rw != 8 && rw != 10) || (post != 0 && post != 2) || !tile_up_fits(rw, depth, levels) || depth < 2) return -1;
+        if (g.TH < 8 || g.TW < 8 || g.tiles_y < 1) return -1;
+        const dim3 grid(g.tiles_y * g.tiles_x), block(kTileWideWaves * kWave);
+        auto go = [&](auto rwc, auto dc, auto pc) {
+            hipLaunchKernelGGL((k_tile_up<T, SM, AR, decltype(rwc)::value, decltype(dc)::value, decltype(pc)::value>), grid, block, 0, st,
+                               a, N, levels, c0, c1, g.tiles_x);
+        };
+        auto with_post = [&](auto rwc, auto dc) {
+            if (post == 2) go(rwc, dc, std::integral_constant<int, 2>{}); else go(rwc, dc, std::integral_constant<int, 0>{});
+        };
+        auto with_depth = [&](auto rwc) {
+            if (depth == 3) with_post(rwc, std::integral_constant<int, 3>{}); else with_post(rwc, std::integral_constant<int, 2>{});
+        };
+        if (rw == 8) with_depth(std::integral_constant<int, 8>{}); else with_depth(std::integral_constant<int, 10>{});
+        return g.tiles_y * g.tiles_x;
+    } else {
+        return -1;
+    }
+}
+
 template <typename T>
 void launch_restrict(const T* v, const T* b, T* cb, T* czero, int N, long pitch, long cpitch,
                      int crow_lo, int crow_hi, int fine_row_off, int mode, bool fused, int rpc, hipStream_t st)
@@ -308,10 +334,13 @@
     extern template bool launch_fused<T, SM, AR>(int, const T*, const T*, T*, int, long, int, int, T, T, int, int, int, int, hipStream_t, int, int);
 #define MGX_DECL_TILE(T, SM, AR) \
     extern template int launch_tile_pass<T, SM, AR>(const T*, const T*, T*, const FoldArgs&, int, long, T, T, int, int, bool, int, hipStream_t);
+#define MGX_DECL_TILE_UP(T, SM, AR) \
+    extern template int launch_tile_up<T, SM, AR>(const TileUpArgs<T>&, int, T, T, int, int, int, int, hipStream_t);
 #if !defined(MGX_INST_KIND) && !defined(MGX_SINGLE_TU)
 MGX_FOR_SMAR(MGX_DECL_CYCLE, double) MGX_FOR_SMAR(MGX_DECL_CYCLE, float)
 MGX_FOR_SMAR(MGX_DECL_FUSED, double) MGX_FOR_SMAR(MGX_DECL_FUSED, float)
 MGX_FOR_SMAR(MGX_DECL_TILE, double) MGX_FOR_SMAR(MGX_DECL_TILE, float)
+MGX_FOR_SMAR(MGX_DECL_TILE_UP, double)
 #endif
 
 }
diff --git a/multigrid_nikhil_c-_amd/csrc/mgx_pass_plan.hpp b/multigrid_nikhil_c-_amd/csrc/mgx_pass_plan.hpp
--- a/multigrid_nikhil_c-_amd/csrc/mgx_pass_plan.hpp
+++ b/multigrid_nikhil_c-_amd/csrc/mgx_pass_plan.hpp
@@ -18,6 +18,7 @@
 struct FuseCfg {
     int kmax; int rows; int min_n; int fold_kmax; int fold_kmax_big; int tile_max_n; int tile_k; int fold_kmax_nopost;
     int tile_wide; int tile_short_n;
+    int up_fuse = 3;
     int plan_pre[8] = {0}; int n_pre = 0; int plan_post[8] = {0}; int n_post = 0; int plan_min_n = 8192;
     int arith = 0;
 };
@@ -74,6 +75,7 @@
     f.tile_short_n = env_int("MGX_TILE_SHORT_N", 512);
     f.tile_max_n = std::max(0, env_int("MGX_TILE_MAX_N", 1024));
     f.tile_k = std::max(2, std::min(10, env_int("MGX_TILE_K", 10)));
+    f.up_fuse = std::max(0, std::min(kTileUpMaxDepth, env_int("MGX_UP_FUSE", kTileUpMaxDepth)));
     f.fold_kmax_nopost = std::max(1, std::min(f.kmax, env_int("MGX_FOLD_KMAX_NOPOST", 10)));
     auto parse = [](const char* name, int* out) {
         const char* v = std::getenv(name);
@@ -264,4 +266,24 @@
     return true;
 }
 
-}
+inline bool up_fuse_stage(const std::vector<Pass>& plan, int N, bool top)
+{
+    if (plan.size() != 1) return false;
+    const Pass& p = plan[0];
+    return p.kind == PASS_TILE && (p.R == 8 || p.R == 10) && p.pre && !p.zero_in && (p.post == 0 || (top && p.post == 2)) &&
+           p.lo == 1 && p.hi == N;
+}
+
+inline int up_fuse_depth(const FuseCfg& fc, const std::vector<Pass>* plans, int n, int N)
+{
+    const int cap = std::min(std::min(fc.up_fuse, kTileUpMaxDepth), n);
+    if (cap < 2 || !up_fuse_stage(plans[0], N, true)) return 1;
+    const Pass& top = plans[0][0];
+    const TileWideGeom g = tile_wide_geom(N, 1, N, top.K + (top.post == 2 ? 1 : 0), 2, top.R);
+    if (g.TH < 8 || g.TW < 8 || g.tiles_y < 1) return 1;
+    int d = 1;
+    while (d < cap && up_fuse_stage(plans[d], N >> d, false) && plans[d][0].K == top.K && tile_up_fits(top.R, d + 1, top.K)) ++d;
+    return d;
+}
+
+}
diff --git a/multigrid_nikhil_c-_amd/csrc/mgx_phase_trace.hpp b/multigrid_nikhil_c-_amd/csrc/mgx_phase_trace.hpp
--- a/multigrid_nikhil_c-_amd/csrc/mgx_phase_trace.hpp
+++ b/multigrid_nikhil_c-_amd/csrc/mgx_phase_trace.hpp
@@ -34,12 +34,19 @@
     }
 }
 
+struct PhaseRef { long long* t; int* n; };
+
 }
 #define MGX_PHASE_BEGIN() __shared__ long long ph_t[mgx::kPhaseMax]; int ph_n = 0; mgx::phase_mark(ph_t, ph_n)
+#define MGX_PHASE_REF() (mgx::PhaseRef{ph_t, &ph_n})
+#define MGX_PHASE_USE(r) long long* const ph_t = (r).t; int& ph_n = *(r).n
 #define MGX_PHASE() mgx::phase_mark(ph_t, ph_n)
 #define MGX_PHASE_AFTER(v) mgx::phase_mark_after(ph_t, ph_n, (v))
 #define MGX_PHASE_END(kind, tag) (mgx::phase_mark(ph_t, ph_n), mgx::phase_flush(ph_t, ph_n, (kind), (tag)))
 #else
+namespace mgx { struct PhaseRef {}; }
+#define MGX_PHASE_REF() (mgx::PhaseRef{})
+#define MGX_PHASE_USE(r) ((void)(r))
 #define MGX_PHASE_BEGIN() ((void)0)
 #define MGX_PHASE() ((void)0)
 #define MGX_PHASE_AFTER(v) ((void)0)
```

Result: no change. 1173 billion, median of 5 (+0.7%).
